# Fadi987/PL-BERT

Measured on AMD Instinct MI355X. Metric: phoneme-tokens/sec, higher is better.
Workload: dtype bf16; 1 GPU; PL-BERT masked-phoneme training step (fwd+loss+bwd+allreduce+AdamW), ALBERT hidden 768 / 12 shared layers / FFN 2048 / 12 heads, seq_len 512, batch 32 per GPU; global_batch=32, seq_len=512, parallelism=dp1

## Files before the change

include/plbert.h:

```cpp
#ifndef PLBERT_H
#define PLBERT_H

#include <stdint.h>

#ifdef __cplusplus
extern "C" {
#endif

typedef struct PlbEngine PlbEngine;

typedef struct {
  int32_t vocab_size;
  int32_t embedding_size;
  int32_t hidden_size;
  int32_t num_attention_heads;
  int32_t intermediate_size;
  int32_t num_hidden_layers;
  int32_t max_position_embeddings;
  int32_t type_vocab_size;
  float layer_norm_eps;
  int32_t num_phonemes;
  int32_t num_tokens;
  int32_t max_batch;
  int32_t max_seq;
// ... 50 lines not shown

int plb_loss_fwd_bwd(PlbEngine* e, const int64_t* masked_ids, const int64_t* labels, const int32_t* lengths,
                     const int32_t* idx_offsets, const int32_t* idx_flat, int32_t n_masked, int32_t B, int32_t S,
                     float* loss, void* stream);

int plb_loss_fwd(PlbEngine* e, const int64_t* masked_ids, const int64_t* labels, const int64_t* token_ids,
                 const int32_t* lengths, const int32_t* idx_offsets, const int32_t* idx_flat, int32_t n_masked, int32_t B,
                 int32_t S, float* loss, float* loss_parts, void* stream);

int plb_loss_fwd_bwd_dual(PlbEngine* e, const int64_t* masked_ids, const int64_t* labels, const int64_t* token_ids,
                          const int32_t* lengths, const int32_t* idx_offsets, const int32_t* idx_flat, int32_t n_masked,
                          int32_t B, int32_t S, float* loss, float* loss_parts, void* stream);

int plb_adamw_step(PlbEngine* e, double lr, double beta1, double beta2, double eps, double weight_decay, int32_t step,
                   double grad_scale, void* stream);

int plb_set_fp8(PlbEngine* e, int32_t on, void* stream);
int plb_fp8_state(const PlbEngine* e, int32_t* enabled, int32_t* calibrated);
int plb_fp8_stats(PlbEngine* e, float clamped_calls[8], float worst_overshoot[8], void* stream);

int32_t plb_token_head_steps(const PlbEngine* e);
int plb_set_token_head_steps(PlbEngine* e, int32_t steps);

#define PLB_COMM_ID_BYTES 128
int plb_comm_unique_id(uint8_t id[PLB_COMM_ID_BYTES]);
int plb_comm_init(PlbEngine* e, const uint8_t id[PLB_COMM_ID_BYTES], int32_t rank, int32_t world);
int plb_comm_destroy(PlbEngine* e);
int plb_comm_info(const PlbEngine* e, int32_t* rank, int32_t* world, int32_t* rccl_version);
int plb_status(PlbEngine* e, int32_t* ln_exchange_timeouts);
int plb_status_ex(PlbEngine* e, int32_t* ln_exchange_timeouts, int32_t* skipped_updates);
int plb_poll_status(const PlbEngine* e, int32_t* ln_exchange_timeouts);
int plb_status_export(PlbEngine* e, float* out, void* stream);
int plb_status_import(PlbEngine* e, const float* summed, void* stream);
int plb_last_application_rows(const PlbEngine* e, int64_t* rows, int64_t* of);
typedef struct {
  const int32_t* row_start;
  int32_t rows;
  int32_t used;
} PlbPacking;
int plb_packing_plan(const int32_t* lengths, int32_t B, int32_t S, int32_t* row_start, int32_t* rows, int32_t* used);
int plb_forward_packed(PlbEngine* e, const int64_t* ids, const int32_t* lengths, int32_t B, int32_t S,
                       const PlbPacking* packing, float* hidden, float* phoneme_logits, float* token_logits, void* stream);
int plb_loss_fwd_bwd_packed(PlbEngine* e, const int64_t* masked_ids, const int64_t* labels, const int32_t* lengths,
                            const int32_t* idx_offsets, const int32_t* idx_flat, int32_t n_masked, int32_t B, int32_t S,
                            const PlbPacking* packing, float* loss, void* stream);
int plb_loss_fwd_packed(PlbEngine* e, const int64_t* masked_ids, const int64_t* labels, const int64_t* token_ids,
                        const int32_t* lengths, const int32_t* idx_offsets, const int32_t* idx_flat, int32_t n_masked,
                        int32_t B, int32_t S, const PlbPacking* packing, float* loss, float* loss_parts, void* stream);
int plb_last_call_rows(const PlbEngine* e, int64_t* rows, int64_t* of);
int plb_encode(PlbEngine* e, const int64_t* ids, const int32_t* lengths, int32_t B, int32_t S, const PlbPacking* packing,
               float* hidden, void* stream);
int plb_encode_bwd(PlbEngine* e, const int64_t* ids, const int32_t* lengths, int32_t B, int32_t S, const PlbPacking* packing,
                   const float* d_hidden, void* stream);
int plb_comm_pieces(const PlbEngine* e, int32_t* collectives, int64_t* floats);
int plb_broadcast_params(PlbEngine* e, int32_t root, void* stream);
int plb_set_grad_overlap(PlbEngine* e, int32_t overlap);
int plb_allreduce_grads(PlbEngine* e, void* stream);

int plb_apply_mask(const int64_t* ids, const int32_t* sample_off, const int32_t* word_off, const int32_t* word_begin,
                   const int32_t* word_len, const int8_t* action, const int64_t* repl, const int64_t* word_token,
                   int64_t sep_token, const int32_t* crop_start, int32_t B, int32_t S, int32_t mask_id, int64_t* labels,
                   int64_t* masked, int64_t* tokens, int32_t* lengths_out, int32_t* idx_offsets, int32_t* idx_flat,
                   int32_t* scratch, void* stream);

int plb_mask_batch(const int64_t* labels, const int32_t* lengths, int32_t B, int32_t S, uint64_t seed, uint32_t step,
                   float word_pred_prob, float phoneme_mask_prob, float replace_prob, int32_t mask_id, int32_t sep_id,
                   int64_t* masked, int32_t* idx_offsets, int32_t* idx_flat, int32_t* scratch, void* stream);

void plb_profile_enable(int on);
int plb_profile_num_classes(void);
const char* plb_profile_class_name(int cls);
int plb_profile_read(double* ms, int64_t* launches, double* flops, double* bytes);

void plb_debug_skip_piece(int index);
void plb_debug_ln_fault(int mode, int launches);
int plb_debug_hb_audit(PlbEngine* e, int32_t on, int32_t break_wait);
int plb_debug_hb_report(const PlbEngine* e, int64_t* checks, int32_t* violations, char* first, int32_t first_bytes);
int plb_comm_trace(PlbEngine* e, int32_t on);
int plb_comm_trace_read(PlbEngine* e, int32_t max_pieces, int32_t* n, int64_t* begin, int64_t* end, float* released_ms,
                        float* done_ms, float* tail_ms);
void plb_set_gemm_nt_tile(int tile);
void plb_set_gemm_nt_prefetch(int on);
void plb_set_attn_bwd_fused(int on);
void plb_set_prune_last(int on);

#ifdef __cplusplus
}
#endif
#endif
```

plbert_amd/_lib.py:

```python
from __future__ import annotations

import ctypes as C
import os

import torch

HERE = os.path.dirname(os.path.abspath(__file__))
LIB_PATH = os.environ.get("PLBERT_HIP_LIB") or os.path.join(HERE, "libplbert_hip.so")

PLB_PARAM_NAMES = [
    "encoder.embeddings.word_embeddings.weight",
    "encoder.embeddings.position_embeddings.weight",
    "encoder.embeddings.token_type_embeddings.weight",
    "encoder.embeddings.LayerNorm.weight",
    "encoder.embeddings.LayerNorm.bias",
    "encoder.encoder.embedding_hidden_mapping_in.weight",
    "encoder.encoder.embedding_hidden_mapping_in.bias",
    "encoder.encoder.albert_layer_groups.0.albert_layers.0.full_layer_layer_norm.weight",
    "encoder.encoder.albert_layer_groups.0.albert_layers.0.full_layer_layer_norm.bias",
    "encoder.encoder.albert_layer_groups.0.albert_layers.0.attention.query.weight",
    "encoder.encoder.albert_layer_groups.0.albert_layers.0.attention.key.weight",
    "encoder.encoder.albert_layer_groups.0.albert_layers.0.attention.value.weight",
    "encoder.encoder.albert_layer_groups.0.albert_layers.0.attention.query.bias",
    "encoder.encoder.albert_layer_groups.0.albert_layers.0.attention.key.bias",
    "encoder.encoder.albert_layer_groups.0.albert_layers.0.attention.value.bias",
    "encoder.encoder.albert_layer_groups.0.albert_layers.0.attention.dense.weight",
    "encoder.encoder.albert_layer_groups.0.albert_layers.0.attention.dense.bias",
    "encoder.encoder.albert_layer_groups.0.albert_layers.0.attention.LayerNorm.weight",
    "encoder.encoder.albert_layer_groups.0.albert_layers.0.attention.LayerNorm.bias",
    "encoder.encoder.albert_layer_groups.0.albert_layers.0.ffn.weight",
    "encoder.encoder.albert_layer_groups.0.albert_layers.0.ffn.bias",
    "encoder.encoder.albert_layer_groups.0.albert_layers.0.ffn_output.weight",
    "encoder.encoder.albert_layer_groups.0.albert_layers.0.ffn_output.bias",
    "phoneme_predictor.weight",
    "phoneme_predictor.bias",
    "encoder.pooler.weight",
    "encoder.pooler.bias",
    "token_predictor.weight",
    "token_predictor.bias",
]
PLB_NPARAM = len(PLB_PARAM_NAMES)

PUBLIC_SYMBOLS = [
    "plb_last_error", "plb_create", "plb_destroy", "plb_param_layout", "plb_workspace_bytes", "plb_bind",
    "plb_sync_weights", "plb_forward", "plb_pooler", "plb_loss_fwd_bwd", "plb_loss_fwd", "plb_loss_fwd_bwd_dual", "plb_adamw_step",
    "plb_set_fp8", "plb_fp8_state", "plb_fp8_stats", "plb_token_head_steps", "plb_set_token_head_steps", "plb_comm_unique_id", "plb_comm_init", "plb_comm_destroy",
    "plb_comm_info", "plb_comm_pieces", "plb_last_application_rows", "plb_last_call_rows",
    "plb_packing_plan", "plb_forward_packed", "plb_loss_fwd_bwd_packed", "plb_loss_fwd_packed", "plb_encode", "plb_encode_bwd", "plb_status", "plb_status_ex", "plb_poll_status", "plb_status_export", "plb_status_import", "plb_broadcast_params", "plb_set_grad_overlap", "plb_allreduce_grads", "plb_apply_mask",
    "plb_mask_batch", "plb_profile_enable", "plb_profile_num_classes", "plb_profile_class_name", "plb_profile_read",
    "plb_debug_skip_piece", "plb_debug_ln_fault", "plb_debug_hb_audit", "plb_debug_hb_report", "plb_comm_trace", "plb_comm_trace_read",
    "plb_set_gemm_nt_tile", "plb_set_gemm_nt_prefetch", "plb_set_attn_bwd_fused", "plb_set_prune_last",
]


class PlbConfig(C.Structure):
    _fields_ = [
        ("vocab_size", C.c_int32), ("embedding_size", C.c_int32), ("hidden_size", C.c_int32),
        ("num_attention_heads", C.c_int32), ("intermediate_size", C.c_int32), ("num_hidden_layers", C.c_int32),
        ("max_position_embeddings", C.c_int32), ("type_vocab_size", C.c_int32), ("layer_norm_eps", C.c_float),
        ("num_phonemes", C.c_int32), ("num_tokens", C.c_int32), ("max_batch", C.c_int32), ("max_seq", C.c_int32),
        ("inference_only", C.c_int32),
    ]


class PlbGemmNT(C.Structure):
    _fields_ = [
        ("A", C.c_void_p), ("lda", C.c_int), ("B", C.c_void_p), ("ldb", C.c_int),
        ("M", C.c_int), ("N", C.c_int), ("K", C.c_int), ("Mstore", C.c_int),
        ("bias", C.c_void_p), ("res", C.c_void_p), ("ldr", C.c_int), ("aux", C.c_void_p), ("ldaux", C.c_int),
        ("C", C.c_void_p), ("ldc", C.c_int), ("C2", C.c_void_p), ("ldc2", C.c_int), ("Cf", C.c_void_p), ("ldcf", C.c_int),
        ("colpart", C.c_void_p),
        ("ce_cols", C.c_int), ("ce_tgt", C.c_void_p), ("ce_pmax", C.c_void_p), ("ce_psum", C.c_void_p),
        ("ce_tlogit", C.c_void_p), ("ce_lse", C.c_void_p), ("ce_w", C.c_void_p),
        ("deq_a", C.c_void_p), ("deq_b", C.c_void_p), ("C8", C.c_void_p), ("ldc8", C.c_int), ("q_scale", C.c_void_p),
        ("q_amax", C.c_void_p), ("c8_bf8", C.c_int),
        ("ln_gamma", C.c_void_p), ("ln_beta", C.c_void_p), ("ln_mean", C.c_void_p), ("ln_rstd", C.c_void_p),
        ("ln_eps", C.c_float), ("ln_xchg", C.c_void_p), ("ln_err", C.c_void_p), ("ln_fault", C.c_int),
    ]


class PlbGemmTN(C.Structure):
    _fields_ = [
        ("A", C.c_void_p), ("lda", C.c_int), ("Ncols", C.c_int), ("B", C.c_void_p), ("ldb", C.c_int),
        ("Mtot", C.c_int), ("N", C.c_int), ("K", C.c_int), ("rows_per_split", C.c_int), ("splits", C.c_int),
        ("slab", C.c_void_p), ("deq_a", C.c_void_p), ("deq_b", C.c_void_p),
    ]


class PlbAttn(C.Structure):
    _fields_ = [
        ("qkv", C.c_void_p), ("ldqkv", C.c_int), ("lengths", C.c_void_p),
        ("B", C.c_int), ("S", C.c_int), ("NH", C.c_int), ("H", C.c_int), ("scale", C.c_float),
        ("ctx", C.c_void_p), ("ldctx", C.c_int), ("lse", C.c_void_p),
        ("dctx", C.c_void_p), ("lddctx", C.c_int), ("delta", C.c_void_p), ("dqkv", C.c_void_p), ("lddqkv", C.c_int),
        ("colpart", C.c_void_p), ("colpart_accumulate", C.c_int),
        ("ctx8", C.c_void_p), ("ldctx8", C.c_int), ("ctx_scale", C.c_void_p), ("ctx_amax", C.c_void_p),
        ("dqkv8", C.c_void_p), ("lddqkv8", C.c_int), ("dqkv_scale", C.c_void_p), ("dqkv_amax", C.c_void_p),
        ("qoff", C.c_void_p), ("q", C.c_void_p), ("ldq", C.c_int), ("nq_total", C.c_int), ("dq", C.c_void_p), ("lddq", C.c_int),
        ("dq8", C.c_void_p), ("lddq8", C.c_int),
        ("row_start", C.c_void_p),
    ]


class PlbEmbed(C.Structure):
    _fields_ = [
        ("ids", C.c_void_p), ("T", C.c_int), ("S", C.c_int), ("E", C.c_int), ("V", C.c_int),
        ("word", C.c_void_p), ("pos", C.c_void_p), ("type0", C.c_void_p), ("gamma", C.c_void_p), ("beta", C.c_void_p),
        ("eps", C.c_float), ("out", C.c_void_p), ("ldo", C.c_int), ("dout", C.c_void_p), ("lddo", C.c_int),
        ("dx", C.c_void_p), ("dword", C.c_void_p), ("dpos", C.c_void_p), ("partials", C.c_void_p), ("nblocks", C.c_int),
        ("row_start", C.c_void_p), ("lengths", C.c_void_p), ("B", C.c_int),
    ]


class PlbPacking(C.Structure):
    _fields_ = [("row_start", C.c_void_p), ("rows", C.c_int32), ("used", C.c_int32)]


class PlbLayerNorm(C.Structure):
    _fields_ = [
        ("x", C.c_void_p), ("ldx", C.c_int), ("gamma", C.c_void_p), ("beta", C.c_void_p), ("eps", C.c_float),
        ("y", C.c_void_p), ("ldy", C.c_int), ("mean", C.c_void_p), ("rstd", C.c_void_p),
        ("T", C.c_int), ("H", C.c_int), ("Tzero", C.c_int),
        ("dy", C.c_void_p), ("lddy", C.c_int), ("dx", C.c_void_p), ("lddx", C.c_int),
        ("partials", C.c_void_p), ("nblocks", C.c_int), ("accumulate", C.c_int),
        ("out8", C.c_void_p), ("ld8", C.c_int), ("q_scale", C.c_void_p), ("q_amax", C.c_void_p),
    ]


_lib = None


class HipLibraryMissing(RuntimeError):
    pass

# ... 18 lines not shown
    L.plb_destroy.restype = None
    L.plb_destroy.argtypes = [vp]
    L.plb_param_layout.restype = C.c_int
    L.plb_param_layout.argtypes = [vp, i64p, i64p, i64p, i64p]
    L.plb_workspace_bytes.restype = C.c_int64
    L.plb_workspace_bytes.argtypes = [vp]
    L.plb_bind.restype = C.c_int
    L.plb_bind.argtypes = [vp, vp, vp, vp, vp, vp, C.c_int64]
    L.plb_sync_weights.restype = C.c_int
    L.plb_sync_weights.argtypes = [vp, vp]
    L.plb_forward.restype = C.c_int
    L.plb_forward.argtypes = [vp, vp, vp, i32, i32, vp, vp, vp, vp]
    L.plb_loss_fwd_bwd.restype = C.c_int
    L.plb_loss_fwd_bwd.argtypes = [vp, vp, vp, vp, vp, vp, i32, i32, i32, vp, vp]
    L.plb_loss_fwd_bwd_dual.restype = C.c_int
    L.plb_loss_fwd_bwd_dual.argtypes = [vp, vp, vp, vp, vp, vp, vp, i32, i32, i32, vp, vp, vp]
    L.plb_pooler.restype = C.c_int
    L.plb_pooler.argtypes = [vp, vp, i32, i32, vp, vp]
    L.plb_loss_fwd.restype = C.c_int
    L.plb_loss_fwd.argtypes = [vp, vp, vp, vp, vp, vp, vp, i32, i32, i32, vp, vp, vp]
    L.plb_set_fp8.restype = C.c_int
    L.plb_set_fp8.argtypes = [vp, i32, vp]
    L.plb_fp8_state.restype = C.c_int
    L.plb_fp8_state.argtypes = [vp, C.POINTER(i32), C.POINTER(i32)]
    L.plb_token_head_steps.restype = i32
    L.plb_token_head_steps.argtypes = [vp]
    L.plb_set_token_head_steps.restype = C.c_int
    L.plb_set_token_head_steps.argtypes = [vp, i32]
    L.plb_comm_unique_id.restype = C.c_int
    L.plb_comm_unique_id.argtypes = [vp]
    L.plb_comm_init.restype = C.c_int
    L.plb_comm_init.argtypes = [vp, vp, i32, i32]
    L.plb_comm_destroy.restype = C.c_int
    L.plb_comm_destroy.argtypes = [vp]
    L.plb_comm_info.restype = C.c_int
    L.plb_comm_info.argtypes = [vp, C.POINTER(i32), C.POINTER(i32), C.POINTER(i32)]
    L.plb_status.restype = C.c_int
    L.plb_status.argtypes = [vp, C.POINTER(i32)]
    L.plb_status_ex.restype = C.c_int
    L.plb_status_ex.argtypes = [vp, C.POINTER(i32), C.POINTER(i32)]
    L.plb_poll_status.restype = C.c_int
    L.plb_poll_status.argtypes = [vp, C.POINTER(i32)]
    L.plb_fp8_stats.restype = C.c_int
    L.plb_fp8_stats.argtypes = [vp, C.POINTER(f32), C.POINTER(f32), vp]
    L.plb_last_application_rows.restype = C.c_int
    L.plb_last_application_rows.argtypes = [vp, i64p, i64p]
    if hasattr(L, "plb_packing_plan"):
        pk = C.POINTER(PlbPacking)
        L.plb_last_call_rows.restype = C.c_int
        L.plb_last_call_rows.argtypes = [vp, i64p, i64p]
        L.plb_packing_plan.restype = C.c_int
        L.plb_packing_plan.argtypes = [vp, i32, i32, vp, C.POINTER(i32), C.POINTER(i32)]
        L.plb_forward_packed.restype = C.c_int
        L.plb_forward_packed.argtypes = [vp, vp, vp, i32, i32, pk, vp, vp, vp, vp]
        L.plb_loss_fwd_bwd_packed.restype = C.c_int
        L.plb_loss_fwd_bwd_packed.argtypes = [vp, vp, vp, vp, vp, vp, i32, i32, i32, pk, vp, vp]
        L.plb_loss_fwd_packed.restype = C.c_int
        L.plb_loss_fwd_packed.argtypes = [vp, vp, vp, vp, vp, vp, vp, i32, i32, i32, pk, vp, vp, vp]
        L.plb_launch_ce_prepare_packed.restype = C.c_int
        L.plb_launch_ce_prepare_packed.argtypes = [vp, vp, vp, C.c_int, C.c_int, vp, vp, vp, vp, vp]
        L.plb_launch_unpack_rows.restype = C.c_int
        L.plb_launch_unpack_rows.argtypes = [vp, C.c_int, C.c_int, vp, vp, C.c_int, C.c_int, C.c_int, vp, vp]
    if hasattr(L, "plb_encode"):
        L.plb_encode.restype = C.c_int
        L.plb_encode.argtypes = [vp, vp, vp, i32, i32, C.POINTER(PlbPacking), vp, vp]
        L.plb_encode_bwd.restype = C.c_int
        L.plb_encode_bwd.argtypes = [vp, vp, vp, i32, i32, C.POINTER(PlbPacking), vp, vp]
        L.plb_launch_seed_dy.restype = C.c_int
        L.plb_launch_seed_dy.argtypes = [vp, vp, vp, C.c_int, C.c_int, C.c_int, C.c_int, vp, vp]
    L.plb_status_export.restype = C.c_int
    L.plb_status_export.argtypes = [vp, vp, vp]
    L.plb_status_import.restype = C.c_int
    L.plb_status_import.argtypes = [vp, vp, vp]
    L.plb_debug_hb_audit.restype = C.c_int
    L.plb_debug_hb_audit.argtypes = [vp, i32, i32]
    L.plb_debug_hb_report.restype = C.c_int
    L.plb_debug_hb_report.argtypes = [vp, i64p, C.POINTER(i32), C.c_char_p, i32]
    L.plb_comm_trace.restype = C.c_int
    L.plb_comm_trace.argtypes = [vp, i32]
    L.plb_comm_trace_read.restype = C.c_int
    L.plb_comm_trace_read.argtypes = [vp, i32, C.POINTER(i32), i64p, i64p, C.POINTER(f32), C.POINTER(f32), C.POINTER(f32)]
    L.plb_debug_ln_fault.restype = None
    L.plb_debug_ln_fault.argtypes = [C.c_int, C.c_int]
    L.plb_debug_skip_piece.restype = None
    L.plb_debug_skip_piece.argtypes = [C.c_int]
    L.plb_comm_pieces.restype = C.c_int
    L.plb_comm_pieces.argtypes = [vp, C.POINTER(i32), C.POINTER(C.c_int64)]
    L.plb_broadcast_params.restype = C.c_int
    L.plb_broadcast_params.argtypes = [vp, i32, vp]
    L.plb_set_grad_overlap.restype = C.c_int
    L.plb_set_grad_overlap.argtypes = [vp, i32]
    L.plb_allreduce_grads.restype = C.c_int
    L.plb_allreduce_grads.argtypes = [vp, vp]
    L.plb_apply_mask.restype = C.c_int
    L.plb_apply_mask.argtypes = [vp, vp, vp, vp, vp, vp, vp, vp, C.c_int64, vp, i32, i32, i32, vp, vp, vp, vp, vp, vp, vp, vp]
    L.plb_adamw_step.restype = C.c_int
    L.plb_adamw_step.argtypes = [vp, f64, f64, f64, f64, f64, i32, f64, vp]
    L.plb_mask_batch.restype = C.c_int
    L.plb_mask_batch.argtypes = [vp, vp, i32, i32, C.c_uint64, C.c_uint32, f32, f32, f32, i32, i32, vp, vp, vp, vp, vp]
    L.plb_profile_enable.restype = None
    L.plb_profile_enable.argtypes = [C.c_int]
    L.plb_profile_num_classes.restype = C.c_int
    L.plb_profile_num_classes.argtypes = []
    L.plb_profile_class_name.restype = C.c_char_p
    L.plb_profile_class_name.argtypes = [C.c_int]
    L.plb_profile_read.restype = C.c_int
    L.plb_profile_read.argtypes = [C.POINTER(C.c_double), i64p, C.POINTER(C.c_double), C.POINTER(C.c_double)]
    L.plb_launch_gemm_nt.restype = C.c_int
    L.plb_launch_gemm_nt.argtypes = [C.POINTER(PlbGemmNT), C.c_int, C.c_int, vp]
    L.plb_set_gemm_nt_tile.restype = None
    L.plb_set_gemm_nt_tile.argtypes = [C.c_int]
    L.plb_set_gemm_nt_prefetch.restype = None
    L.plb_set_gemm_nt_prefetch.argtypes = [C.c_int]
    L.plb_launch_gemm_nt_fp8.restype = C.c_int
    L.plb_launch_gemm_nt_fp8.argtypes = [C.POINTER(PlbGemmNT), C.c_int, C.c_int, vp]
    L.plb_launch_gemm_nt_fp8_ln.restype = C.c_int
    L.plb_launch_gemm_nt_fp8_ln.argtypes = [C.POINTER(PlbGemmNT), C.c_int, C.c_int, vp]
    L.plb_launch_gemm_nt_fp8_gelud.restype = C.c_int
    L.plb_launch_gemm_nt_fp8_gelud.argtypes = [C.POINTER(PlbGemmNT), C.c_int, C.c_int, vp]
    L.plb_launch_gemm_tn.restype = C.c_int
    L.plb_launch_gemm_tn.argtypes = [C.POINTER(PlbGemmTN), vp]
    L.plb_launch_gemm_tn_big.restype = C.c_int
    L.plb_launch_gemm_tn_big.argtypes = [C.POINTER(PlbGemmTN), vp]
    L.plb_launch_gemm_tn_fp8.restype = C.c_int
    L.plb_launch_gemm_tn_fp8.argtypes = [C.POINTER(PlbGemmTN), vp]
    L.plb_launch_reduce_slabs.restype = C.c_int
    L.plb_launch_reduce_slabs.argtypes = [vp, C.c_int, C.c_size_t, vp, C.c_int, vp]
    L.plb_launch_attn_fwd.restype = C.c_int
    L.plb_launch_attn_fwd.argtypes = [C.POINTER(PlbAttn), vp]
    L.plb_launch_gemm_nt_ln.restype = C.c_int
    L.plb_launch_gemm_nt_ln.argtypes = [C.POINTER(PlbGemmNT), C.c_int, vp]
    L.plb_launch_gemm_nt_gelud.restype = C.c_int
    L.plb_launch_gemm_nt_gelud.argtypes = [C.POINTER(PlbGemmNT), C.c_int, vp]
    L.plb_launch_attn_bwd.restype = C.c_int
    L.plb_launch_attn_bwd.argtypes = [C.POINTER(PlbAttn), vp]
    L.plb_launch_attn_bwd_fused.restype = C.c_int
    L.plb_launch_attn_bwd_fused.argtypes = [C.POINTER(PlbAttn), vp]
    L.plb_set_prune_last.restype = None
    L.plb_set_prune_last.argtypes = [C.c_int]
    L.plb_set_attn_bwd_fused.restype = None
    L.plb_set_attn_bwd_fused.argtypes = [C.c_int]
    L.plb_launch_ln_fwd.restype = C.c_int
    L.plb_launch_ln_fwd.argtypes = [C.POINTER(PlbLayerNorm), vp]
    L.plb_launch_ln_bwd.restype = C.c_int
    L.plb_launch_ln_bwd.argtypes = [C.POINTER(PlbLayerNorm), vp]
    L.plb_launch_embed_scatter.restype = C.c_int
    L.plb_launch_embed_scatter.argtypes = [C.POINTER(PlbEmbed), C.c_int, vp]
    L.plb_launch_ce_prepare.restype = C.c_int
    L.plb_launch_ce_prepare.argtypes = [vp, vp, vp, C.c_int, C.c_int, vp, vp, vp, vp]
    L.plb_launch_colsum.restype = C.c_int
    L.plb_launch_colsum.argtypes = [vp, C.c_int, C.c_size_t, C.c_int, C.c_int, vp, C.c_int, C.c_int, vp, C.c_int, vp]
    _lib = L
    return L


def profile_enable(on):
    lib().plb_profile_enable(int(bool(on)))


def profile_read():
    L = lib()
    n = L.plb_profile_num_classes()
    ms, fl, by = (C.c_double * n)(), (C.c_double * n)(), (C.c_double * n)()
    cnt = (C.c_int64 * n)()
    check(L.plb_profile_read(ms, cnt, fl, by), "plb_profile_read")
    return {L.plb_profile_class_name(i).decode(): dict(ms=ms[i], launches=int(cnt[i]), flops=fl[i], bytes=by[i])
# ... 8 lines not shown
```

plbert_amd/csrc/attn_bwd_fused.hip:

```cpp
#include "attn_common.h"

namespace {

constexpr int FB_KIMG = 0;
constexpr int FB_EXCH = 65536;
constexpr int FB_STG = FB_EXCH + 65536;
constexpr int FB_STAT = FB_STG + 16384;
constexpr int FB_TOTAL = FB_STAT + 512;

DEVI int kt_of(int key) { return ((key >> 1) & 1) | (((key >> 3) & 1) << 1); }
DEVI int du_f(int row) { return (((row >> 1) & 1) << 2) | ((row >> 2) & 1) | (((row >> 3) & 1) << 1); }

typedef float f32x4v __attribute__((ext_vector_type(4)));
#define MFMA16(a, b, c) __builtin_amdgcn_mfma_f32_16x16x32_bf16(a, b, c, 0, 0, 0)

DEVI bf16x8 join_tr(s16x4 a, s16x4 b) { return bf16x8{a[0], a[1], a[2], a[3], b[0], b[1], b[2], b[3]}; }
typedef __attribute__((address_space(3))) const bf16x8 lds_cbf16x8;
typedef uint32_t u32x2_t __attribute__((ext_vector_type(2)));
typedef __attribute__((address_space(3))) const f32x4 lds_cf32x4;
typedef __attribute__((address_space(3))) u32x2_t lds_u32x2;
DEVI bf16x8 lds_rd128(uint32_t a) { return *(lds_cbf16x8*)(uintptr_t)a; }
DEVI f32x4 lds_rdf4(uint32_t a) { return *(lds_cf32x4*)(uintptr_t)a; }
DEVI void lds_wr64(uint32_t a, uint32_t x, uint32_t y) { *(lds_u32x2*)(uintptr_t)a = u32x2_t{x, y}; }
DEVI bf16x8 lds_tr2(uint32_t a0, uint32_t a1) { return join_tr(lds_read_tr16_addr(a0), lds_read_tr16_addr(a1)); }
// ... 308 lines not shown
      DQ_PHASE((CUR) ^ 1);                                                                                       \
      DQ_STORE(it_ - 1);                                                                                         \
    }                                                                                                            \
    STAMP(2);                                                                                                    \
    if (it_ + 1 < NQ) F_STAT_STORE((CUR) ^ 1, it_ + 1);                                                          \
    STAMP(3);                                                                                                    \
    DMA_WAIT();                                                                                                  \
    __syncthreads();                                                                                             \
    STAMP(4);                                                                                                    \
  } while (0)
#if FUSED_DBG & 1024
  const unsigned long long tstart_ = __builtin_readcyclecounter();
  tl_ = tstart_;
#endif
  for (int i = 0; i <= NQ; i += 2) {
    F_ITER(0, i);
    if (i + 1 <= NQ) F_ITER(1, i + 1);
  }
#if FUSED_DBG & 1024
  if (lane == 0 && p.delta) {
    float* o_ = p.delta + ((size_t)blockIdx.x * 4 + wave) * 8;
    for (int k = 0; k < 6; ++k) o_[k] = (float)tk_[k] * 1e-3f;
    o_[6] = (float)(tl_ - tstart_) * 1e-3f;
  }
#endif

  LANE_ID(lane_e);
  const int tid_e = wave * 64 + lane_e;
  for (int r = NQ * 32 + (tid_e >> 3); r < S; r += 32) {
    if (B16) *(uint4*)(p.dqkv + (tok0 + r) * p.lddqkv + hd * 64 + (tid_e & 7) * 8) = make_uint4(0, 0, 0, 0);
    if (F8) *(uint2*)(p.dqkv8 + (tok0 + r) * p.lddqkv8 + hd * 64 + (tid_e & 7) * 8) = make_uint2(0, 0);
  }
  bf16_t* patch = (bf16_t*)(smem + FB_EXCH) + wave * (32 * 72);
  const bool accq = p.colpart_accumulate != 0;
#pragma unroll
  for (int kb = 0; kb < 4; ++kb) {
    const int key0 = wave * 128 + kb * 32;
    int rows_valid = S - key0; rows_valid = rows_valid > 32 ? 32 : rows_valid;
    float* cp = (p.colpart && wave < QT) ? p.colpart + ((size_t)(b * QT + wave) * 4 + kb) * (3 * H) + hd * 64 : nullptr;
    if (rows_valid > 0) {
      bf16_t* out = B16 ? p.dqkv + (tok0 + key0) * p.lddqkv + hd * 64 : nullptr;
      uint8_t* out8 = F8 ? p.dqkv8 + (tok0 + key0) * p.lddqkv8 + hd * 64 : nullptr;
      const Out8 ok8 = {out8 ? out8 + H : nullptr, p.lddqkv8, qs8, true}, ov8 = {out8 ? out8 + 2 * H : nullptr, p.lddqkv8, qs8, true};
      store_transposed<false, true>(dk[kb][0], dk[kb][1], p.scale, patch, out ? out + H : nullptr, p.lddqkv, rows_valid, lane_e,
                                    cp ? cp + H : nullptr, accq, F8 ? &ok8 : nullptr, &amax8);
      __builtin_amdgcn_wave_barrier();
      store_transposed<false, true>(dv[kb][0], dv[kb][1], 1.0f, patch, out ? out + 2 * H : nullptr, p.lddqkv, rows_valid, lane_e,
                                    cp ? cp + 2 * H : nullptr, accq, F8 ? &ov8 : nullptr, &amax8);
      __builtin_amdgcn_wave_barrier();
    } else if (cp && !accq) {
      cp[H + lane_e] = 0.f;
      cp[2 * H + lane_e] = 0.f;
    }
  }
  if (F8 && p.dqkv_amax) {
    amax8 = wave_max(amax8);
    if (lane_e == 0) atomic_max_abs(p.dqkv_amax, amax8, blockIdx.x * 4 + wave);
  }
  if (p.colpart) {
#pragma unroll
    for (int r = 0; r < 4; ++r) {
      float v = colq[r];
      v += __shfl_xor(v, 1, 64); v += __shfl_xor(v, 2, 64); v += __shfl_xor(v, 4, 64); v += __shfl_xor(v, 8, 64);
      colq[r] = v;
    }
    float* row0 = p.colpart + (size_t)(b * QT) * 4 * (3 * H) + hd * 64;
    if ((lane_e & 15) == 0) {
      float* d = row0 + 16 * wave + 4 * (lane_e >> 4);
#pragma unroll
      for (int r = 0; r < 4; ++r) d[r] = accq ? d[r] + colq[r] : colq[r];
    }
    if (!accq)
      for (int rr = 1 + wave; rr < 4 * QT; rr += 4) row0[(size_t)rr * (3 * H) + lane_e] = 0.f;
  }
}

}

extern "C" int plb_launch_attn_bwd_fused(const PlbAttn* p, hipStream_t stream) {
  if (p->H != p->NH * 64 || p->S < 1 || p->S > 512 || p->B < 1) return 1;
  if (p->row_start && !p->lengths) return 1;
  if (p->ldqkv % 8 || p->ldctx % 8 || p->lddctx % 8 || p->lddqkv % 8) return 1;
  if ((!p->dqkv && !p->dqkv8) || (p->dqkv8 && (!p->dqkv_scale || p->lddqkv8 % 8))) return 1;
  dim3 grid(p->NH * p->B), block(256);
  const double unit = (double)p->B * p->NH * (double)p->S * p->S * 64.0;
  const double io = 2.0 * p->B * p->S * (double)p->H;
  const int tok = plb_prof_begin(PLB_K_ATTN_BWD, stream, 8.0 * unit, 6.0 * io);
  if (p->dqkv && p->dqkv8) return 1;
  if (!p->dqkv8) hipLaunchKernelGGL(attn_bwd_fused_kernel<0>, grid, block, 0, stream, *p);
  else hipLaunchKernelGGL(attn_bwd_fused_kernel<1>, grid, block, 0, stream, *p);
  plb_prof_end(tok, stream);
  return hipGetLastError() == hipSuccess ? 0 : 2;
}
```

plbert_amd/csrc/engine.cpp:

```cpp
#include <stdarg.h>

#include <new>

#include "engine_internal.h"

static thread_local char g_err[512] = "";
int fail(const char* fmt, ...) {
  va_list ap;
  va_start(ap, fmt);
  vsnprintf(g_err, sizeof(g_err), fmt, ap);
  va_end(ap);
  return 1;
}
extern "C" const char* plb_last_error(void) { return g_err; }

static void layout_params(PlbEngine* e) {
  const int64_t V = e->V, E = e->E, H = e->H, I = e->I, P = e->P, NP = e->NP, NT = e->NT;
  int64_t sz[PLB_NPARAM];
  sz[PLB_WORD_EMB] = V * E; sz[PLB_POS_EMB] = P * E; sz[PLB_TYPE_EMB] = (int64_t)e->c.type_vocab_size * E;
  sz[PLB_EMB_LN_W] = E; sz[PLB_EMB_LN_B] = E;
  sz[PLB_MAP_W] = H * E; sz[PLB_MAP_B] = H;
  sz[PLB_LN2_W] = H; sz[PLB_LN2_B] = H;
  sz[PLB_Q_W] = sz[PLB_K_W] = sz[PLB_V_W] = H * H;
  sz[PLB_Q_B] = sz[PLB_K_B] = sz[PLB_V_B] = H;
// ... 23 lines not shown
    return o;
  }
};
}

extern "C" int plb_create(const PlbConfig* cfg, PlbEngine** out) {
  if (!cfg || !out) return fail("plb_create: null argument");
  const PlbConfig& c = *cfg;
  if (c.hidden_size != c.num_attention_heads * 64) return fail("plb_create: head_dim must be 64 (hidden %d, heads %d)", c.hidden_size, c.num_attention_heads);
  if (c.embedding_size % 64 || c.embedding_size > 256) return fail("plb_create: embedding_size must be a multiple of 64, <= 256");
  if (c.hidden_size % 128 || c.hidden_size > 1024) return fail("plb_create: hidden_size must be a multiple of 128, <= 1024");
  if (c.intermediate_size % 128) return fail("plb_create: intermediate_size must be a multiple of 128");
  if (c.num_phonemes < 4 || c.num_phonemes % 4 || c.num_phonemes > 256) return fail("plb_create: num_phonemes must be a multiple of 4 in [4,256]");
  if (c.num_tokens < 0 || c.num_tokens % 4) return fail("plb_create: num_tokens must be a non-negative multiple of 4");
  if (c.max_seq < 1 || c.max_seq > c.max_position_embeddings) return fail("plb_create: max_seq must be in [1, max_position_embeddings]");
  if (c.max_batch < 1 || c.num_hidden_layers < 1 || c.vocab_size < 1 || c.type_vocab_size < 1) return fail("plb_create: bad sizes");
  PlbEngine* e = new (std::nothrow) PlbEngine();
  if (!e) return fail("plb_create: out of host memory");
  e->c = c;
  e->E = c.embedding_size; e->H = c.hidden_size; e->I = c.intermediate_size; e->L = c.num_hidden_layers;
  e->NH = c.num_attention_heads; e->V = c.vocab_size; e->P = c.max_position_embeddings;
  e->NP = c.num_phonemes; e->NT = c.num_tokens;
  layout_params(e);
  const int64_t E = e->E, H = e->H, I = e->I, L = e->L;
  const int64_t T = (int64_t)c.max_batch * c.max_seq;
  const int64_t Tp = rup(T, 128);
  e->infer = c.inference_only != 0;
  const bool tr = !e->infer;
  const int64_t Ls = tr ? L : 1;
  e->Tcap = Tp;
  e->NMcap = Tp;
  e->ln_blocks = 512;
  if (const char* v = getenv("PLBERT_LN_BLOCKS")) { const int n = atoi(v); if (n >= 64 && n <= 4096) e->ln_blocks = n; }
  e->emb_blocks = 2048;
  if (const char* v = getenv("PLBERT_LN_FUSE"))
    e->ln_fuse = !strcmp(v, "off") ? 0 : !strcmp(v, "fwd") ? 1 : !strcmp(v, "bwd") ? 2 : 3;
  e->part_rows = e->ln_blocks > (int)(2 * Tp / 128) ? e->ln_blocks : (int)(2 * Tp / 128);
  if (const char* v = getenv("PLBERT_GELU_STASH")) e->gelu_dstash_on = strcmp(v, "u") != 0;
  if (const char* v = getenv("PLBERT_FP8_TN")) e->fp8_tn = strcmp(v, "0") != 0;
  if (const char* v = getenv("PLBERT_HB_AUDIT")) e->hb.on = strcmp(v, "0") != 0;
  Carve cv;
  e->o_wbf = cv.take((e->ptotal + 256 * (H > I ? H : I)) * 2);
  if (tr) {
    e->o_wqkvT = cv.take(rup(H, 128) * 3 * H * 2);
    e->o_wdT = cv.take(rup(H, 128) * H * 2);
    e->o_w1T = cv.take(rup(H, 128) * I * 2);
    e->o_w2T = cv.take(rup(I, 128) * H * 2);
    e->o_wpT = cv.take(rup(H, 128) * 256 * 2);
    e->o_winT = cv.take(rup(E, 128) * H * 2);
  }
  e->o_e = cv.take(Tp * E * 2);
  e->o_x = cv.take((tr ? L + 1 : 2) * Tp * H * 2);
  e->o_qkv = cv.take(Ls * Tp * 3 * H * 2);
  e->o_ctx = cv.take(Ls * Tp * H * 2);
  e->o_pre1 = cv.take(Ls * Tp * H * 2);
  e->o_a = cv.take(Ls * Tp * H * 2);
  e->o_u = cv.take(Ls * Tp * I * 2);
  e->o_g = cv.take(Ls * Tp * I * 2);
  e->o_pre2 = cv.take(Ls * Tp * H * 2);
  const int64_t stat = (int64_t)c.max_batch * e->NH * c.max_seq * 4;
  e->o_lse = cv.take(Ls * stat);
  e->o_mean1 = cv.take(Ls * Tp * 4); e->o_rstd1 = cv.take(Ls * Tp * 4);
  e->o_mean2 = cv.take(Ls * Tp * 4); e->o_rstd2 = cv.take(Ls * Tp * 4);
  e->lnx_bytes = (Tp / 128) * 16 * 128 * 2 * 8;
  e->o_lnx = cv.take(e->lnx_bytes);
  e->o_lnerr = cv.take(256);
  if (tr) {
    e->o_delta = cv.take(stat);
    e->o_dqkv = cv.take(L * Tp * 3 * H * 2);
    e->o_dpre1 = cv.take(L * Tp * H * 2);
    e->o_du = cv.take(L * Tp * I * 2);
    e->o_dpre2 = cv.take(L * Tp * H * 2);
    e->o_dy0 = cv.take(Tp * H * 2); e->o_dy1 = cv.take(Tp * H * 2);
    e->o_da = cv.take(Tp * H * 2); e->o_dctx = cv.take(Tp * H * 2);
    e->o_de = cv.take(Tp * E * 2);
  }
  const int64_t NM = e->NMcap;
  e->o_hm = cv.take(NM * H * 2);
  e->o_logm = cv.take(NM * 256 * 4);
  e->o_dlog = cv.take(NM * 256 * 2);
  e->o_rows = cv.take(NM * 4); e->o_tgt = cv.take(NM * 4); e->o_w = cv.take(NM * 4); e->o_lrows = cv.take(NM * 4);
  if (tr) {
    e->o_dhm = cv.take(NM * H * 2);
    int64_t slab = 0;
    {
      const int64_t Mtot = L * Tp;
      const int ntp = (int)rup(e->NT, 256);
      const int shapes[7][2] = {{(int)(3 * H), (int)H}, {(int)H, (int)H}, {(int)I, (int)H}, {(int)H, (int)I}, {(int)H, (int)E}, {e->NP, (int)H}, {ntp, (int)H}};
      for (int i = 0; i < (e->NT ? 7 : 6); ++i) {
        int rps;
        const int64_t mt = i < 4 ? Mtot : Tp;
        const int s = tn_splits(mt, shapes[i][0], shapes[i][1], &rps);
        const int64_t f = (int64_t)s * shapes[i][0] * shapes[i][1];
        if (f > slab) slab = f;
      }
    }
    e->slab_floats = slab;
    e->o_slab = cv.take(slab * 4);
    e->o_part1 = cv.take(L * e->part_rows * 3 * H * 4);
    e->o_part2 = cv.take(L * e->part_rows * 3 * H * 4);
    e->o_parte = cv.take((int64_t)e->emb_blocks * 2 * E * 4);
    e->o_dxe = cv.take(Tp * E * 4);
    e->o_ducol = cv.take(L * (2 * Tp / 128) * I * 4);
    e->qkvcol_rows = c.max_batch * ((c.max_seq + 127) / 128) * 4;
    e->o_qkvcol = cv.take((int64_t)L * e->qkvcol_rows * 3 * H * 4);
    e->o_scratch = cv.take(512 * (3 * H > I ? 3 * H : I) * 4);
    e->o_scratch2 = cv.take(512 * (3 * H > I ? 3 * H : I) * 4);
    {
      int rps;
      const int s2 = tn_splits(Tp, (int)H, (int)E, &rps);
      e->slab2_floats = (int64_t)s2 * H * E;
      e->o_slab2 = cv.take(e->slab2_floats * 4);
    }
  }
  if (e->NT) {
    const int64_t NTp = rup(e->NT, 256);
    e->NTp = (int)NTp;
    e->o_bt = cv.take(NTp * 4);
    e->o_tlrows = cv.take(Tp * 4);
    e->o_tpmax = cv.take(Tp * (NTp / 256) * 4);
    e->o_tpsum = cv.take(Tp * (NTp / 256) * 4);
    e->o_ttl = cv.take(Tp * 4); e->o_tlse = cv.take(Tp * 4); e->o_tw = cv.take(Tp * 4);
    e->o_ttgt = cv.take(Tp * 8);
    e->o_tloss = cv.take(256);
    if (tr) {
      e->o_wtT = cv.take(rup(H, 128) * NTp * 2);
      e->o_tdl = cv.take(Tp * NTp * 2);
      e->o_tscr = cv.take(32 * NTp * 4);
      e->o_tcolp = cv.take(2 * (Tp / 128) * NTp * 4);
      e->o_tgrad = cv.take(NTp * H * 4);
    }
  }
  e->o_x8 = cv.take(Ls * Tp * H); e->o_a8 = cv.take(Ls * Tp * H); e->o_g8 = cv.take(Ls * Tp * I); e->o_c8 = cv.take(Ls * Tp * H);
  e->o_wq8 = cv.take(rup(3 * H, 128) * H + 256 * H);
  e->o_wd8 = cv.take(rup(H, 128) * H + 256 * H);
  e->o_w18 = cv.take(rup(I, 128) * H + 256 * H);
  e->o_w28 = cv.take(rup(H, 128) * I + 256 * I);
  if (tr) {
    e->o_dp8 = cv.take(L * Tp * H); e->o_du8 = cv.take(L * Tp * I); e->o_dp18 = cv.take(L * Tp * H); e->o_dq8 = cv.take(L * Tp * 3 * H);
    e->o_w2T8 = cv.take(rup(I, 128) * H + 256 * H);
    e->o_w1T8 = cv.take(rup(H, 128) * I + 256 * I);
    e->o_wqT8 = cv.take(rup(H, 128) * 3 * H + 256 * 3 * H);
    e->o_wdT8 = cv.take(rup(H, 128) * H + 256 * H);
  }
  e->f8n = 8 * (int)L + 8;
  e->o_f8amax = cv.take((int64_t)e->f8n * 64 * 16 * 4); e->o_f8scale = cv.take(e->f8n * 4); e->o_f8deq = cv.take(e->f8n * 4);
  e->o_f8stats = cv.take(8 * 8 * 4);
  e->ws_bytes = cv.off;
  *out = e;
  return 0;
}

extern "C" void plb_destroy(PlbEngine* e) {
  if (!e) return;
  (void)plb_comm_destroy(e);
  if (e->ev_fork) (void)hipEventDestroy(e->ev_fork);
  if (e->ev_join) (void)hipEventDestroy(e->ev_join);
  if (e->side) (void)hipStreamDestroy(e->side);
  if (e->host_err) (void)hipHostFree(e->host_err);
  for (auto& t : e->trace) { (void)hipEventDestroy(t.released); (void)hipEventDestroy(t.done); }
  for (auto ev : e->trace_pool) (void)hipEventDestroy(ev);
  for (auto ev : {e->tr_call0, e->tr_tail0, e->tr_tail1}) if (ev) (void)hipEventDestroy(ev);
  delete e;
}

extern "C" int plb_param_layout(const PlbEngine* e, int64_t* offsets, int64_t* sizes, int64_t* total, int64_t* trainable) {
  if (!e) return fail("plb_param_layout: null engine");
  for (int i = 0; i < PLB_NPARAM; ++i) {
    if (offsets) offsets[i] = e->poff[i];
    if (sizes) sizes[i] = e->psize[i];
  }
  if (total) *total = e->ptotal;
  if (trainable) *trainable = e->ptrain;
  return 0;
}

extern "C" int64_t plb_workspace_bytes(const PlbEngine* e) { return e ? e->ws_bytes : -1; }

extern "C" int plb_bind(PlbEngine* e, float* params, float* grads, float* exp_avg, float* exp_avg_sq, void* workspace,
                        int64_t workspace_bytes) {
  if (!e || !params || !workspace) return fail("plb_bind: null argument");
  if (workspace_bytes < e->ws_bytes) return fail("plb_bind: workspace too small (%lld < %lld)", (long long)workspace_bytes, (long long)e->ws_bytes);
  if (((uintptr_t)params | (uintptr_t)grads | (uintptr_t)exp_avg | (uintptr_t)exp_avg_sq) & 15) return fail("plb_bind: buffers must be 16-byte aligned");
  if ((uintptr_t)workspace & 255) return fail("plb_bind: workspace must be 256-byte aligned");
  e->params = params; e->grads = grads; e->m = exp_avg; e->v = exp_avg_sq;
  e->ws = (char*)workspace;
  if (!e->host_err) {
    void* h = nullptr;
    if (hipHostMalloc(&h, 64, hipHostMallocMapped) == hipSuccess && h) {
      void* d = nullptr;
      if (hipHostGetDevicePointer(&d, h, 0) == hipSuccess && d) {
        e->host_err = (unsigned int*)h;
        e->host_err_dev = (unsigned int*)d;
        *e->host_err = 0;
      } else {
        (void)hipHostFree(h);
      }
    }
    if (!e->host_err) return fail("plb_bind: cannot allocate the pinned status word");
  }
  if (!e->side && grads && !getenv("PLBERT_NO_SIDE_STREAM")) {
    if (hipStreamCreateWithFlags(&e->side, hipStreamNonBlocking) != hipSuccess) e->side = nullptr;
    if (e->side && (hipEventCreateWithFlags(&e->ev_fork, kStreamOrderEvent) != hipSuccess ||
                    hipEventCreateWithFlags(&e->ev_join, kStreamOrderEvent) != hipSuccess)) {
      (void)hipStreamDestroy(e->side);
      e->side = nullptr;
    }
  }
  return 0;
}

static int sync_transposes(PlbEngine* e, hipStream_t s, bool exact_fp8 = true) {
  const int H = e->H, I = e->I, E = e->E;

  if (e->NT) {
    if (!e->tok_pad_zeroed) HIPTRY(hipMemsetAsync(e->at<float>(e->o_bt), 0, (size_t)e->NTp * 4, s));
    HIPTRY(hipMemcpyAsync(e->at<float>(e->o_bt), e->par(PLB_TOK_B), (size_t)e->NT * 4, hipMemcpyDeviceToDevice, s));
  }
  if (e->infer) {
    e->tok_pad_zeroed = true;
    if (e->fp8_on) return fp8_quantize_weights(e, s, exact_fp8 || e->fp8_wstale);
    return 0;
  }
  const float* tsrc[8] = {e->par(PLB_Q_W), e->par(PLB_DENSE_W), e->par(PLB_FFN_W), e->par(PLB_FFNO_W), e->par(PLB_HEAD_W),
                          e->par(PLB_MAP_W)};
  bf16_t* tdst[8] = {e->at<bf16_t>(e->o_wqkvT), e->at<bf16_t>(e->o_wdT), e->at<bf16_t>(e->o_w1T), e->at<bf16_t>(e->o_w2T),
                     e->at<bf16_t>(e->o_wpT), e->at<bf16_t>(e->o_winT)};
  int tR[8] = {3 * H, H, I, H, e->NP, H}, tC[8] = {H, H, H, I, H, E}, tld[8] = {3 * H, H, I, H, 256, H};
  int nt = 6;
  if (e->NT) {
    if (!e->tok_pad_zeroed) HIPTRY(hipMemsetAsync(e->at<bf16_t>(e->o_wtT), 0, (size_t)rup(H, 128) * e->NTp * 2, s));
    tsrc[nt] = e->par(PLB_TOK_W); tdst[nt] = e->at<bf16_t>(e->o_wtT); tR[nt] = e->NT; tC[nt] = H; tld[nt] = e->NTp;
    ++nt;
  }
  TRY(plb_launch_transpose_cast_multi(nt, tsrc, tR, tC, tdst, tld, s));
  e->tok_pad_zeroed = true;
  if (e->fp8_on) return fp8_quantize_weights(e, s, exact_fp8 || e->fp8_wstale);
  return 0;
}

extern "C" int plb_sync_weights(PlbEngine* e, void* stream) {
  if (!e || !e->ws) return fail("plb_sync_weights: engine not bound");
  drop_stash(e, "plb_sync_weights refreshed the compute copies since");
  hipStream_t s = (hipStream_t)stream;
  TRY(plb_launch_cast_bf16(e->params, e->at<bf16_t>(e->o_wbf), (size_t)e->ptotal, s));
  return sync_transposes(e, s);
}

extern "C" int plb_pooler(PlbEngine* e, const float* hidden, int32_t B, int32_t S, float* pooled, void* stream) {
  if (!e || !e->ws) return fail("plb_pooler: engine not bound");
  if (!hidden || !pooled || B < 1 || S < 1) return fail("plb_pooler: bad argument");
  TRY(plb_launch_pooler(hidden, B, S, e->H, e->par(PLB_POOL_W), e->par(PLB_POOL_B), pooled, (hipStream_t)stream));
  return 0;
}

#ifndef PLB_PACK_GRAN_MAX
#define PLB_PACK_GRAN_MAX 1024
#endif
extern "C" int plb_packing_plan(const int32_t* lengths, int32_t B, int32_t S, int32_t* row_start, int32_t* rows,
                                int32_t* used) {
// ... 112 lines not shown
```

plbert_amd/csrc/engine_calls.cpp:

```cpp
#include "engine_internal.h"

void drop_stash(PlbEngine* e, const char* by) {
  if (e && e->stash_live) { e->stash_live = false; e->stash_dead_by = by; }
}

static int check_shape(const PlbEngine* e, int B, int S, const char* who) {
  if (!e || !e->ws) return fail("%s: engine not bound", who);
  if (B < 1 || S < 1 || B > e->c.max_batch || S > e->c.max_seq || (int64_t)B * S > (int64_t)e->c.max_batch * e->c.max_seq)
    return fail("%s: batch %d x seq %d exceeds the engine capacity %d x %d", who, B, S, e->c.max_batch, e->c.max_seq);
  return 0;
}

static Rows padded_rows(int B, int S) { return Rows{nullptr, B * S, rup(B * S, 128)}; }
static int pick_rows(PlbEngine* e, const PlbPacking* pk, const int32_t* lengths, bool dual, int B, int S, const char* who,
                     Rows* out) {
  *out = padded_rows(B, S);
  e->last_exec_rows[0] = e->last_exec_rows[1] = (int64_t)B * S;
  if (!pk || !pk->row_start) return 0;
  if (pk->rows < 128 || pk->rows % 128 || pk->used < 1 || pk->used > pk->rows)
    return fail("%s: packing plan of %d rows (%d used) is not one plb_packing_plan made", who, pk->rows, pk->used);
  if (pk->rows > out->Tp) return fail("%s: packing plan of %d rows exceeds the call's %lld", who, pk->rows, (long long)out->Tp);
  if (!lengths || dual || e->fp8_on || pk->rows == out->Tp) return 0;
  if (pk->used % 128) return fail("%s: packing plan with %d used rows: slots are multiples of 128", who, pk->used);
  *out = Rows{pk->row_start, pk->used, pk->rows};
// ... 225 lines not shown
  } else {
    HB_R(s2, st.du, Mtot_c * I * 2, "dU of every application");
    TRY(plb_launch_colsum(st.du, 1, (size_t)Mtot_c, I, I, e->grd(PLB_FFN_B), I, 0, scratch2, 64, s2));
  }
  const size_t prow = (size_t)L * e->part_rows_used;
  HB_R(s2, st.part1, (int64_t)L * e->part_rows * 3 * H * 4, "LayerNorm-1 backward partial rows");
  HB_W(s2, e->grd(PLB_DENSE_B), 3 * H * 4, "dense.bias + LayerNorm-1 affine gradients");
  TRY(plb_launch_colsum(st.part1, 0, prow, 3 * H, 3 * H, e->grd(PLB_LN1_W), 2 * H, 0, scratch2, 64, s2));
  TRY(plb_launch_copy_cols(scratch2, 64, 3 * H, 2 * H, H, e->grd(PLB_DENSE_B), s2));
  HB_R(s2, st.part2, (int64_t)L * e->part_rows * 3 * H * 4, "LayerNorm-2 backward partial rows");
  HB_W(s2, e->grd(PLB_LN2_W), 2 * H * 4, "LayerNorm-2 affine gradients"); HB_W(s2, e->grd(PLB_FFNO_B), H * 4, "ffn_output.bias gradient");
  TRY(plb_launch_colsum(st.part2, 0, prow, 3 * H, 3 * H, e->grd(PLB_LN2_W), 2 * H, 0, scratch2, 64, s2));
  TRY(plb_launch_copy_cols(scratch2, 64, 3 * H, 2 * H, H, e->grd(PLB_FFNO_B), s2));
  if (s2 != s) HIPTRY(ev_record(e, e->ev_join, s2));
  const bool ov = overlapping(e);
  const bool t8 = e->tn8_call;
  float* const slab = e->at<float>(e->o_slab);
  HB_W(s, slab, e->slab_floats * 4, "weight-gradient slab"); HB_W(s, e->grd(PLB_Q_W), 3 * H * H * 4, "Q/K/V weight gradients");
  if (t8 ? weight_grad8(e, st.dq8, st.x8, Mtot, 3 * H, H, F8_DQ, F8_X, e->grd(PLB_Q_W), s)
         : weight_grad(e, st.dqkv, 3 * H, 3 * H, st.x, H, Mtot, 3 * H, H, e->grd(PLB_Q_W), s)) return 1;
  if (ov && reduce_pieces(e, kPieceQkvW, kPieceFfnW, s)) return 1;
  HB_W(s, slab, e->slab_floats * 4, "weight-gradient slab"); HB_W(s, e->grd(PLB_FFN_W), (int64_t)I * H * 4, "ffn.weight gradient");
  if (t8 ? weight_grad8(e, st.du8, st.a8, Mtot_c, I, H, F8_DU, F8_A, e->grd(PLB_FFN_W), s)
         : weight_grad(e, st.du, I, I, st.a, H, Mtot_c, I, H, e->grd(PLB_FFN_W), s)) return 1;
  if (ov && reduce_pieces(e, kPieceFfnW, kPieceSmall, s)) return 1;
  if (ov) {
    if (reduce_pieces(e, kPieceSmall, kPieceFfnoW, s2)) return 1;
  }
  HB_W(s, slab, e->slab_floats * 4, "weight-gradient slab"); HB_W(s, e->grd(PLB_FFNO_W), (int64_t)I * H * 4, "ffn_output.weight gradient");
  if (t8 ? weight_grad8(e, st.dp8, st.g8, Mtot_c, H, I, F8_DP, F8_G, e->grd(PLB_FFNO_W), s)
         : weight_grad(e, st.dpre2, H, H, st.g, I, Mtot_c, H, I, e->grd(PLB_FFNO_W), s)) return 1;
  if (ov && reduce_pieces(e, kPieceFfnoW, kPieceDenseW, s)) return 1;
  HB_W(s, slab, e->slab_floats * 4, "weight-gradient slab"); HB_W(s, e->grd(PLB_DENSE_W), (int64_t)H * H * 4, "dense.weight gradient");
  if (t8 ? weight_grad8(e, st.dp18, st.c8, Mtot_c, H, H, F8_DP1, F8_C, e->grd(PLB_DENSE_W), s)
         : weight_grad(e, st.dpre1, H, H, st.ctx, H, Mtot_c, H, H, e->grd(PLB_DENSE_W), s)) return 1;
  if (ov && reduce_pieces(e, kPieceDenseW, kNPieces, s)) return 1;
  return 0;
}

static int backward_tail(PlbEngine* e, const int64_t* masked_ids, const int32_t* lengths, bf16_t* dy, int B, int S,
                         const Rows& rw, int du_rows, hipStream_t s) {
  hipStream_t s2 = s;
  float* scratch2 = e->at<float>(e->o_scratch);
  HB_W(s, e->ws, e->ws_bytes, "layer loop (whole workspace)");
  if (e->trace_on) (void)hipEventRecord(e->tr_tail0, s);
  if (e->side) {
    s2 = e->side;
    scratch2 = e->at<float>(e->o_scratch2);
    HIPTRY(ev_record(e, e->ev_fork, s));
    HIPTRY(ev_wait(e, s2, e->ev_fork));
  }
  const int rc = backward_tail_streams(e, masked_ids, lengths, dy, B, S, rw, du_rows, s, s2, scratch2);
  if (s2 != s) {
    if (rc) (void)ev_record(e, e->ev_join, s2);
    const hipError_t je = ev_wait(e, s, e->ev_join);
    if (!rc && je != hipSuccess) return fail("plb_loss_fwd_bwd: joining the side stream: %s", hipGetErrorString(je));
  }
  if (e->trace_on) { (void)hipEventRecord(e->tr_tail1, s); e->tr_tail_valid = true; }
  if (rc) return rc;
  HB_W(s, e->ws, e->ws_bytes, "after the side stream's join (whole workspace)");
  return pieces_done(e);
}

static int loss_impl(PlbEngine* e, bool backward, const int64_t* masked_ids, const int64_t* labels,
                     const int64_t* token_targets, const int32_t* lengths, const int32_t* idx_offsets,
                     const int32_t* idx_flat, int32_t n_masked, int32_t B, int32_t S, const PlbPacking* pk, float* loss,
                     float* loss_parts, void* stream) {
  const char* who = backward ? "plb_loss_fwd_bwd" : "plb_loss_fwd";
  if (check_shape(e, B, S, who)) return 1;
  drop_stash(e, "a plb_loss_* call rewrote the workspace since");
  if (backward && e->infer) return fail("%s: inference-only engine (PlbConfig.inference_only = 1)", who);
  if (backward && !e->grads) return fail("%s: no gradient buffer bound", who);
  if (!masked_ids || !labels || !idx_offsets || !loss) return fail("%s: null argument", who);
  if (n_masked < 0 || n_masked > e->NMcap) return fail("%s: n_masked %d out of range", who, n_masked);
  if (token_targets && !e->NT) return fail("%s: the engine has no token head (num_tokens = 0)", who);
  hipStream_t s = (hipStream_t)stream;
  Rows rw;
  if (pick_rows(e, pk, lengths, token_targets != nullptr, B, S, who, &rw)) return 1;
  const int64_t Tp = rw.Tp;
  if (backward && begin_training_call(e, token_targets != nullptr, s)) return 1;
  if (n_masked == 0 && !token_targets) return zero_loss_call(e, backward, loss, s);

  const int NM = (int)rup(n_masked, 128);
  Prune pr = {e->at<int32_t>(e->o_rows), n_masked, NM};
  const bool prune = prune_enabled() && n_masked > 0 && !token_targets && e->L >= 2 && 2 * (int64_t)NM <= Tp;
  if (n_masked > 0) {
    if (rw.row_start)
      TRY(plb_launch_ce_prepare_packed(idx_offsets, idx_flat, labels, B, S, rw.row_start, e->at<int32_t>(e->o_rows),
                                       e->at<int32_t>(e->o_tgt), e->at<float>(e->o_w), s));
    else
      TRY(plb_launch_ce_prepare(idx_offsets, idx_flat, labels, B, S, e->at<int32_t>(e->o_rows), e->at<int32_t>(e->o_tgt),
                                e->at<float>(e->o_w), s));
  }
  if (backward) e->pruned_rows = prune ? NM : 0;
  e->last_app_rows[0] = prune ? NM : Tp; e->last_app_rows[1] = Tp;
  bf16_t* xL = nullptr;
  if (run_encoder(e, masked_ids, lengths, B, S, rw, backward, &xL, s, prune ? &pr : nullptr)) return 1;
  bf16_t* dy = backward ? e->at<bf16_t>(e->o_dy0) : nullptr;
  if (phoneme_head(e, backward, prune, xL, n_masked, Tp, dy, loss, s)) return 1;
  if (loss_parts) HIPTRY(hipMemcpyAsync(loss_parts, loss, sizeof(float), hipMemcpyDeviceToDevice, s));
  if (token_targets && token_head(e, backward, xL, token_targets, lengths, B, S, dy, loss, loss_parts, s)) return 1;
  if (!backward) {
    if (e->fp8_on) {
      TRY(fp8_update_scales(e, s));
      e->fp8_ready = true;
    }
    e->last_loss = loss;
    TRY(plb_launch_step_status(e->at<unsigned int>(e->o_lnerr), loss, e->host_err_dev, nullptr, s));
    return 0;
  }

  int du_rows = 0;
  if (encoder_bwd(e, prune ? &pr : nullptr, lengths, B, S, rw, &dy, &du_rows, s)) return 1;
  if (status_exchange(e, s)) return 1;
  if (backward_tail(e, masked_ids, lengths, dy, B, S, rw, du_rows, s)) return 1;
  if (e->fp8_on) {
    TRY(fp8_update_scales(e, s));
    e->fp8_ready = true;
    e->fp8_bwd_ready = true;
  }
  return status_finish(e, loss, s);
}

extern "C" int plb_loss_fwd_bwd(PlbEngine* e, const int64_t* masked_ids, const int64_t* labels, const int32_t* lengths,
                                const int32_t* idx_offsets, const int32_t* idx_flat, int32_t n_masked, int32_t B,
                                int32_t S, float* loss, void* stream) {
  return loss_impl(e, true, masked_ids, labels, nullptr, lengths, idx_offsets, idx_flat, n_masked, B, S, nullptr, loss, nullptr,
                   stream);
}
extern "C" int plb_loss_fwd_bwd_packed(PlbEngine* e, const int64_t* masked_ids, const int64_t* labels, const int32_t* lengths,
                                       const int32_t* idx_offsets, const int32_t* idx_flat, int32_t n_masked, int32_t B,
                                       int32_t S, const PlbPacking* packing, float* loss, void* stream) {
  return loss_impl(e, true, masked_ids, labels, nullptr, lengths, idx_offsets, idx_flat, n_masked, B, S, packing, loss, nullptr,
                   stream);
}

extern "C" int plb_loss_fwd_bwd_dual(PlbEngine* e, const int64_t* masked_ids, const int64_t* labels,
                                     const int64_t* token_ids, const int32_t* lengths, const int32_t* idx_offsets,
                                     const int32_t* idx_flat, int32_t n_masked, int32_t B, int32_t S, float* loss,
                                     float* loss_parts, void* stream) {
  if (!token_ids) return fail("plb_loss_fwd_bwd_dual: token_ids is null");
  return loss_impl(e, true, masked_ids, labels, token_ids, lengths, idx_offsets, idx_flat, n_masked, B, S, nullptr, loss,
                   loss_parts, stream);
}

extern "C" int plb_loss_fwd(PlbEngine* e, const int64_t* masked_ids, const int64_t* labels, const int64_t* token_ids,
                            const int32_t* lengths, const int32_t* idx_offsets, const int32_t* idx_flat, int32_t n_masked,
                            int32_t B, int32_t S, float* loss, float* loss_parts, void* stream) {
  return loss_impl(e, false, masked_ids, labels, token_ids, lengths, idx_offsets, idx_flat, n_masked, B, S, nullptr, loss,
                   loss_parts, stream);
}
extern "C" int plb_loss_fwd_packed(PlbEngine* e, const int64_t* masked_ids, const int64_t* labels, const int64_t* token_ids,
                                   const int32_t* lengths, const int32_t* idx_offsets, const int32_t* idx_flat,
                                   int32_t n_masked, int32_t B, int32_t S, const PlbPacking* packing, float* loss,
                                   float* loss_parts, void* stream) {
  return loss_impl(e, false, masked_ids, labels, token_ids, lengths, idx_offsets, idx_flat, n_masked, B, S, packing, loss,
                   loss_parts, stream);
}

extern "C" int plb_encode(PlbEngine* e, const int64_t* ids, const int32_t* lengths, int32_t B, int32_t S,
                          const PlbPacking* pk, float* hidden, void* stream) {
  if (check_shape(e, B, S, "plb_encode")) return 1;
  if (e->infer) return fail("plb_encode: inference-only engine (PlbConfig.inference_only = 1): a differentiable forward keeps every application's activations");
  if (!e->grads) return fail("plb_encode: no gradient buffer bound");
  if (e->fp8_on) return fail("plb_encode: fp8 mode is on (the gradient sites' delayed scales belong to the pre-training loss); call plb_set_fp8(e, 0, stream) first");
  if (!ids || !hidden) return fail("plb_encode: %s is null", !ids ? "ids" : "hidden");
  hipStream_t s = (hipStream_t)stream;
  Rows rw;
  if (pick_rows(e, pk, lengths, false, B, S, "plb_encode", &rw)) return 1;
  drop_stash(e, "a plb_encode call that failed rewrote the workspace since");
  HB_W(s, e->ws, e->ws_bytes, "plb_encode (whole workspace)");
  e->last_app_rows[0] = e->last_app_rows[1] = rw.Tp;
  bf16_t* x = nullptr;
  if (run_encoder(e, ids, lengths, B, S, rw, true, &x, s)) return 1;
  if (lengths) TRY(plb_launch_unpack_rows(x, 1, e->H, rw.row_start, lengths, B, S, e->H, hidden, s));
// ... 47 lines not shown
```

plbert_amd/csrc/engine_internal.h:

```cpp
#pragma once
#include <hip/hip_runtime.h>
#include <stdint.h>
#include <stdio.h>
#include <stdlib.h>
#include <string.h>

#include <array>
#include <map>
#include <string>
#include <vector>

#include "../../include/plbert.h"
#include "plbert_kernels.h"

#pragma GCC visibility push(hidden)

int fail(const char* fmt, ...);

static const unsigned kStreamOrderEvent = hipEventDisableTiming | hipEventReleaseToDevice;

inline int64_t rup(int64_t x, int64_t m) { return (x + m - 1) / m * m; }

#define TRY(x)                                                                    \
  do {                                                                            \
    int rc_ = (x);                                                                \
    if (rc_) return fail("%s failed (rc %d) at %s:%d", #x, rc_, __FILE__, __LINE__); \
  } while (0)
#define HIPTRY(x)                                                                                   \
  do {                                                                                              \
    hipError_t e_ = (x);                                                                            \
    if (e_ != hipSuccess) return fail("%s: %s at %s:%d", #x, hipGetErrorString(e_), __FILE__, __LINE__); \
  } while (0)
#define HB_R(stream, ptr, bytes, what) do { if (e->hb.on) e->hb.access(hb_idx(e, stream), (ptr), (size_t)(bytes), false, what); } while (0)
#define HB_W(stream, ptr, bytes, what) do { if (e->hb.on) e->hb.access(hb_idx(e, stream), (ptr), (size_t)(bytes), true, what); } while (0)

typedef void* RcclComm;

struct HbAudit {
  enum { MAIN = 0, SIDE = 1, COMM = 2, NS = 3 };
  typedef std::array<uint64_t, NS> VC;
  struct Acc { const char* what; uintptr_t a, b; int st; uint64_t tick; bool wr; };
  bool on = false;
  int break_wait = -1;
  int waits = 0;
  VC vc[NS] = {{0, 0, 0}, {0, 0, 0}, {0, 0, 0}};
  std::map<hipEvent_t, VC> ev;
  std::vector<Acc> log;
  int64_t checks = 0;
  int violations = 0;
  std::string first;
  static const char* name(int st) { return st == MAIN ? "main" : st == SIDE ? "side" : "comm"; }
  void record(hipEvent_t e, int st) { vc[st][st] += 1; ev[e] = vc[st]; }
  void wait(int st, hipEvent_t e);
  void access(int st, const void* p, size_t bytes, bool wr, const char* what);
  void new_call() { log.clear(); waits = 0; }
};

struct PlbEngine {
  PlbConfig c;
  int64_t poff[PLB_NPARAM], psize[PLB_NPARAM], ptotal, ptrain;
  int E, H, I, L, NH, V, P, NP, NT;
  int64_t Tcap;
  int64_t NMcap;
  int NTp = 0;
  bool infer = false;
  int qkvcol_rows = 0;
  int64_t slab2_floats;
  int64_t slab_floats;
  int64_t ws_bytes;
  int ln_blocks, emb_blocks;
  int part_rows = 0;
  int ln_fuse = 3;
  int64_t lnx_bytes = 0;
  bool gelu_dstash_on = true;
  bool fp8_tn = true;
  int f8n = 0;
  int64_t o_wbf, o_wqkvT, o_wdT, o_w1T, o_w2T, o_wpT, o_winT;
  int64_t o_e, o_x, o_qkv, o_ctx, o_pre1, o_a, o_u, o_g, o_pre2;
  int64_t o_lse, o_delta, o_mean1, o_rstd1, o_mean2, o_rstd2;
  int64_t o_dqkv, o_dpre1, o_du, o_dpre2;
  int64_t o_dy0, o_dy1, o_da, o_dctx, o_de;
  int64_t o_hm, o_logm, o_dlog, o_dhm, o_rows, o_tgt, o_w, o_lrows;
  int64_t o_slab, o_part1, o_part2, o_parte, o_scratch, o_dxe, o_ducol, o_slab2, o_scratch2, o_qkvcol = 0;
  int64_t o_lnx = 0, o_lnerr = 0;
  int64_t o_bt = 0, o_wtT = 0, o_tdl = 0, o_tlrows = 0, o_tscr = 0, o_tgrad = 0, o_tloss = 0;
  int64_t o_tpmax = 0, o_tpsum = 0, o_ttl = 0, o_tlse = 0, o_tw = 0, o_ttgt = 0, o_tcolp = 0;
  int64_t o_x8 = 0, o_a8 = 0, o_g8 = 0, o_c8 = 0, o_dp8 = 0, o_du8 = 0, o_dp18 = 0, o_dq8 = 0;
  int64_t o_wq8 = 0, o_wd8 = 0, o_w18 = 0, o_w28 = 0, o_w2T8 = 0, o_w1T8 = 0, o_wqT8 = 0, o_wdT8 = 0;
  int64_t o_f8amax = 0, o_f8scale = 0, o_f8deq = 0, o_f8stats = 0;
  bool fp8_on = false, fp8_ready = false, fp8_bwd_ready = false, fp8_wstale = true;
  bool u_is_derivative = false;
  bool tn8_call = false;
  int part_rows_used = 0;
  int pruned_rows = 0;
  int64_t last_app_rows[2] = {0, 0};
  int64_t last_exec_rows[2] = {0, 0};
  bool tok_grads_live = false;
  bool head_grads_live = true;
  bool tok_pad_zeroed = false;
  int tok_steps = 0;
  bool stash_live = false;
  const char* stash_dead_by = "no plb_encode has run on this engine";
  int stash_B = 0, stash_S = 0;
  int64_t stash_rows = 0, stash_used = 0;
  const int32_t* stash_row_start = nullptr;
  RcclComm comm = nullptr;
  int comm_rank = 0, comm_world = 1;
  hipStream_t comm_stream = nullptr;
  hipEvent_t ev_piece = nullptr, ev_comm_done = nullptr;
  bool overlap = true;
  bool comm_pending = false;
  bool grads_reduced = false;
  int64_t piece_floats = 0;
  int32_t piece_count = 0;
  hipEvent_t ev_status = nullptr;
  bool status_pending = false;
  int32_t status_collectives = 0;
  float* last_loss = nullptr;
  HbAudit hb;
  struct PieceTrace { int64_t a, b; hipEvent_t released, done; };
  bool trace_on = false;
  std::vector<PieceTrace> trace;
  std::vector<hipEvent_t> trace_pool;
  hipEvent_t tr_call0 = nullptr, tr_tail0 = nullptr, tr_tail1 = nullptr;
  bool tr_tail_valid = false;
  hipStream_t side = nullptr;
  hipEvent_t ev_fork = nullptr, ev_join = nullptr;
  unsigned int* host_err = nullptr;
  unsigned int* host_err_dev = nullptr;
  float *params = nullptr, *grads = nullptr, *m = nullptr, *v = nullptr;
  char* ws = nullptr;

  template <typename T>
  T* at(int64_t off) const { return reinterpret_cast<T*>(ws + off); }
  bf16_t* wbf(int which) const { return at<bf16_t>(o_wbf) + poff[which]; }
  float* par(int which) const { return params + poff[which]; }
  float* grd(int which) const { return grads + poff[which]; }
};

enum { F8_X = 0, F8_A, F8_G, F8_C, F8_DP, F8_DU, F8_DP1, F8_DQ, F8_NSITE };
enum { F8_AMAX_WORDS = 64 * 16 };
enum { F8W_QKV = 0, F8W_D, F8W_1, F8W_2, F8W_2T, F8W_1T, F8W_QKVT, F8W_DT, F8W_N };

struct Rows {
  const int32_t* row_start;
  int T; int64_t Tp;
};

struct F8Site {
  float* scale = nullptr;
  float* amax = nullptr;
  float* deq = nullptr;
  F8Site() = default;
  F8Site(const PlbEngine* e, int kind, int l);
};
struct F8Weight {
  const uint8_t* img;
  const float* deq;
  F8Weight(const PlbEngine* e, int w);
};

struct F8Op { const uint8_t* A8; const uint8_t* B8; const float* deq_a; const float* deq_b; int a_bf8; };

struct Slots {
  bf16_t *x, *y;
  bf16_t *qkv, *ctx, *pre1, *a, *u, *g, *pre2;
  float *mean1, *rstd1, *mean2, *rstd2, *lse;
  uint8_t *x8, *x8n, *c8, *a8, *g8;
  bf16_t *dqkv, *dpre1, *du, *dpre2;
  uint8_t *dp8, *du8, *dp18, *dq8;
  float *part1, *part2, *qkvcol, *ducol;
};

struct LnSlot { const float* gamma; const float* beta; const bf16_t* pre; float* mean; float* rstd; float* partials; };

struct Prune { const int32_t* rows; int n; int Mc; };

struct Bwd {
  const int32_t* lengths;
  const int32_t* row_start;
  int B, S, T;
  int64_t Tp;
  bool f8, calib;
  bool fuse_b;
  int prows;
  int du_rows;
  hipStream_t s;
};

enum { kPieceHead = 0, kPieceQkvW, kPieceFfnW, kPieceSmall, kPieceFfnoW = kPieceSmall + 5, kPieceDenseW, kNPieces };

int hb_idx(const PlbEngine* e, hipStream_t s);
hipError_t ev_record(PlbEngine* e, hipEvent_t ev, hipStream_t s);
hipError_t ev_wait(PlbEngine* e, hipStream_t s, hipEvent_t ev);
int reduce_piece(PlbEngine* e, int64_t a, int64_t b, hipStream_t after);
bool overlapping(const PlbEngine* e);
int pieces_done(PlbEngine* e);
int64_t piece_begin(const PlbEngine* e, int i);
int64_t piece_end(const PlbEngine* e, int i);
int reduce_pieces(PlbEngine* e, int from, int to, hipStream_t after);
int status_exchange(PlbEngine* e, hipStream_t s);
int status_finish(PlbEngine* e, float* loss, hipStream_t s);
int f8_site(const PlbEngine* e, int site, int l);
float* f8_deq(const PlbEngine* e, int i);
int fp8_quantize_weights(PlbEngine* e, hipStream_t s, bool exact = true);
int fp8_update_scales(PlbEngine* e, hipStream_t s);
bool f8_call(const PlbEngine* e, int64_t Tp, bool train);
bool tn8_ok(const PlbEngine* e, int64_t Mtot);
PlbGemmNT nt_desc(const bf16_t* A, const bf16_t* B, int64_t M, int N, int K);
int qkvcol_rows(int B, int S);
Slots slots(const PlbEngine* e, int64_t Tp, int B, int S, int l, bool stash, int prows = 0, int du_rows = 0);
bool prune_enabled();
int run_encoder(PlbEngine* e, const int64_t* ids, const int32_t* lengths, int B, int S, const Rows& rw, bool stash,
                bf16_t** xout, hipStream_t s, const Prune* pr = nullptr);
int tn_splits(int64_t Mtot, int N, int K, int* rows_per_split);
int weight_grad(PlbEngine* e, const bf16_t* A, int lda, int Ncols, const bf16_t* Bm, int ldb, int64_t Mtot, int N,
                int K, float* out, hipStream_t s, bool side_slab = false);
int weight_grad8(PlbEngine* e, const uint8_t* A8, const uint8_t* B8, int64_t Mtot, int N, int K, int site_a, int site_b,
                 float* out, hipStream_t s);
int encoder_bwd(PlbEngine* e, const Prune* pr, const int32_t* lengths, int B, int S, const Rows& rw, bf16_t** dy,
                int* du_rows, hipStream_t s);
void drop_stash(PlbEngine* e, const char* by);

#pragma GCC visibility pop
```

plbert_amd/csrc/engine_layers.cpp:

```cpp
#include "engine_internal.h"

static bool tn_big(int64_t Mtot, int Ncols, int K) { return Ncols % 256 == 0 && K % 256 == 0 && Mtot >= 8192; }
static bool tn_fill_chip() {
  static const bool v = [] { const char* e = getenv("PLBERT_TN_SPLITS"); return !(e && !strcmp(e, "xcd")); }();
  return v;
}
static int tn_cus() {
  static const int v = [] {
    const char* e = getenv("PLBERT_TN_CUS");
    const int n = e ? atoi(e) : 256;
    return (n >= 64 && n <= 256) ? n : 256;
  }();
  return v;
}
int tn_splits(int64_t Mtot, int N, int K, int* rows_per_split) {
  const bool big = tn_big(Mtot, N, K);
  const int tiles = big ? (N / 256) * (K / 256) : ((N + 127) / 128) * ((K + 127) / 128);
  int splits = 768 / tiles;
  if (big) {
    int s = 32 / tiles;
    if (s < 1) s = 1;
    splits = tiles >= 256 ? 1 : (tn_fill_chip() ? (tn_cus() / tiles > 0 ? tn_cus() / tiles : 1) : 8 * s);
  }
  const int64_t maxs = Mtot / 64;
// ... 58 lines not shown
    v.dqkv = bf(e->o_dqkv, 3 * H); v.dpre1 = bf(e->o_dpre1, H); v.du = bf(e->o_du, I); v.dpre2 = bf(e->o_dpre2, H);
    v.dp8 = u8(e->o_dp8, H); v.du8 = u8(e->o_du8, I); v.dp18 = u8(e->o_dp18, H); v.dq8 = u8(e->o_dq8, 3 * H);
    v.part1 = f32(e->o_part1, (int64_t)prows * 3 * H); v.part2 = f32(e->o_part2, (int64_t)prows * 3 * H);
    v.qkvcol = f32(e->o_qkvcol, (int64_t)qkvcol_rows(B, S) * 3 * H); v.ducol = f32(e->o_ducol, (int64_t)du_rows * I);
  }
  return v;
}

static bool ln_fusable(const PlbEngine* e, int64_t Tp, int bit) {
  const int H = e->H;
  return (e->ln_fuse & bit) && Tp % 1024 == 0 && (H % 384 == 0 ? H / 384 : H % 256 == 0 ? H / 256 : 99) <= 4;
}
static bool gelu_dstash(PlbEngine* e, int64_t Tp, bool f8_call) {
  e->u_is_derivative = e->gelu_dstash_on && (f8_call ? Tp % 128 == 0 : Tp % 256 == 0) && e->I % 256 == 0;
  return e->u_is_derivative;
}
static void ln_fields(const PlbEngine* e, PlbGemmNT* g, const float* gamma, const float* beta, float* mean, float* rstd) {
  g->ln_gamma = gamma; g->ln_beta = beta; g->ln_mean = mean; g->ln_rstd = rstd; g->ln_eps = e->c.layer_norm_eps;
  g->ln_xchg = e->at<unsigned long long>(e->o_lnx); g->ln_err = e->at<unsigned int>(e->o_lnerr);
}
static LnSlot ln1_slot(const PlbEngine* e, const Slots& v) {
  return LnSlot{e->par(PLB_LN1_W), e->par(PLB_LN1_B), v.pre1, v.mean1, v.rstd1, v.part1};
}
static LnSlot ln2_slot(const PlbEngine* e, const Slots& v) {
  return LnSlot{e->par(PLB_LN2_W), e->par(PLB_LN2_B), v.pre2, v.mean2, v.rstd2, v.part2};
}
static int gemm_ln_fwd(PlbEngine* e, PlbGemmNT* g, const F8Op* f8, bool fused, const LnSlot& ln, bf16_t* y, int T,
                       uint8_t* y8, const F8Site& q, hipStream_t s) {
  const int H = e->H;
  if (fused) {
    g->C2 = y; g->ldc2 = H;
    ln_fields(e, g, ln.gamma, ln.beta, ln.mean, ln.rstd);
    if (y8) f8_out(g, y8, H, q, 0);
    TRY(gemm_nt_ln_any(g, 5, f8, s));
    return 0;
  }
  TRY(gemm_nt_any(g, 0, f8, s));
  PlbLayerNorm p;
  memset(&p, 0, sizeof(p));
  p.x = g->C; p.ldx = H; p.gamma = ln.gamma; p.beta = ln.beta; p.eps = e->c.layer_norm_eps;
  p.y = y; p.ldy = H; p.T = T; p.H = H; p.mean = ln.mean; p.rstd = ln.rstd;
  if (y8) { p.out8 = y8; p.ld8 = H; p.q_scale = q.scale; p.q_amax = q.amax; }
  TRY(plb_launch_ln_fwd(&p, s));
  return 0;
}
static int ln_bwd(PlbEngine* e, const LnSlot& ln, int nblocks, const bf16_t* dy, bf16_t* dx, int T, int Tzero, uint8_t* dx8,
                  const F8Site& q, hipStream_t s) {
  const int H = e->H;
  PlbLayerNorm p;
  memset(&p, 0, sizeof(p));
  p.x = ln.pre; p.ldx = H; p.gamma = ln.gamma; p.T = T; p.H = H; p.Tzero = Tzero; p.mean = ln.mean; p.rstd = ln.rstd;
  p.dy = dy; p.lddy = H; p.dx = dx; p.lddx = H; p.partials = ln.partials; p.nblocks = nblocks;
  if (dx8) { p.out8 = dx8; p.ld8 = H; p.q_scale = q.scale; p.q_amax = q.amax; }
  TRY(plb_launch_ln_bwd(&p, s));
  return 0;
}
static int gemm_ln_bwd(PlbEngine* e, PlbGemmNT* g, const F8Op* f8, bool fused, const LnSlot& ln, int nblocks, bf16_t* dx, int T,
                       int Tzero, uint8_t* dx8, const F8Site& q, hipStream_t s) {
  if (fused) {
    g->C = dx; g->aux = ln.pre; g->ldaux = e->H; g->colpart = ln.partials;
    ln_fields(e, g, ln.gamma, nullptr, ln.mean, ln.rstd);
    if (dx8) f8_out(g, dx8, e->H, q, 1);
    TRY(gemm_nt_ln_any(g, 6, f8, s));
    return 0;
  }
  TRY(gemm_nt_any(g, 0, f8, s));
  return ln_bwd(e, ln, nblocks, g->C, dx, T, Tzero, dx8, q, s);
}

static int g_prune_last = -1;
extern "C" void plb_set_prune_last(int on) { g_prune_last = on < 0 ? -1 : (on ? 1 : 0); }
bool prune_enabled() {
  static const bool v = [] { const char* e = getenv("PLBERT_PRUNE_LAST"); return !(e && !strcmp(e, "0")); }();
  return g_prune_last < 0 ? v : g_prune_last != 0;
}
static int last_application_fwd_pruned(PlbEngine* e, const Prune* pr, bool stash, bool calib, bool tn8, const Slots& sl,
                                       const bf16_t* ctx_att, hipStream_t s) {
  const int H = e->H, I = e->I, L = e->L, Mc = pr->Mc, n = pr->n;
  const F8Site sA(e, F8_A, L - 1), sG(e, F8_G, L - 1), sC(e, F8_C, L - 1);
  bf16_t* ctxc = stash ? sl.ctx : sl.pre1;
  bf16_t* xc = stash ? e->at<bf16_t>(e->o_da) : sl.a;
  bf16_t* pre1c = stash ? sl.pre1 : sl.ctx;
  bf16_t* ac = stash ? sl.a : sl.pre1;
  TRY(plb_launch_gather_rows(ctx_att, H, pr->rows, n, Mc, H, ctxc, H, s));
  TRY(plb_launch_gather_rows(sl.x, H, pr->rows, n, Mc, H, xc, H, s));
  PlbGemmNT g = nt_desc(ctxc, e->wbf(PLB_DENSE_W), Mc, H, H);
  g.bias = e->par(PLB_DENSE_B); g.res = xc; g.ldr = H; g.C = pre1c; g.ldc = H;
  const LnSlot ln1 = {e->par(PLB_LN1_W), e->par(PLB_LN1_B), pre1c, sl.mean1, sl.rstd1, nullptr};
  if (gemm_ln_fwd(e, &g, nullptr, false, ln1, ac, Mc, nullptr, F8Site(), s)) return 1;
  if (calib) TRY(plb_launch_amax(ac, 1, (size_t)n, H, H, sA.amax, s));
  g = nt_desc(ac, e->wbf(PLB_FFN_W), Mc, I, H);
  g.bias = e->par(PLB_FFN_B); g.C = sl.u; g.ldc = I; g.C2 = sl.g; g.ldc2 = I;
  TRY(plb_launch_gemm_nt(&g, 1, 0, s));
  if (calib) TRY(plb_launch_amax(sl.g, 1, (size_t)n, I, I, sG.amax, s));
  g = nt_desc(sl.g, e->wbf(PLB_FFNO_W), Mc, H, I);
  g.bias = e->par(PLB_FFNO_B); g.res = ac; g.ldr = H; g.C = sl.pre2; g.ldc = H;
  if (gemm_ln_fwd(e, &g, nullptr, false, ln2_slot(e, sl), e->at<bf16_t>(e->o_hm), Mc, nullptr, F8Site(), s)) return 1;
  if (tn8) {
    const void* src[3] = {ctxc, ac, sl.g}; const int fl[3] = {1, 1, 1};
    const size_t nel[3] = {(size_t)Mc * H, (size_t)Mc * H, (size_t)Mc * I};
    const float* sc[3] = {sC.scale, sA.scale, sG.scale};
    uint8_t* dst[3] = {sl.c8, sl.a8, sl.g8};
    float* am[3] = {sC.amax, sA.amax, sG.amax};
    TRY(plb_launch_quantize_multi(3, src, fl, nel, sc, dst, am, s));
  }
  return 0;
}

int run_encoder(PlbEngine* e, const int64_t* ids, const int32_t* lengths, int B, int S, const Rows& rw, bool stash,
                       bf16_t** xout, hipStream_t s, const Prune* pr) {
  const int E = e->E, H = e->H, I = e->I, L = e->L;
  const int T = rw.T;
  const int64_t Tp = rw.Tp;
  const bool f8 = f8_call(e, Tp, stash);
  const bool calib = e->fp8_on && !f8;
  if (e->fp8_on && e->fp8_wstale) TRY(fp8_quantize_weights(e, s));
  PlbEmbed em;
  memset(&em, 0, sizeof(em));
  em.ids = ids; em.T = T; em.S = S; em.E = E; em.V = e->V;
  em.word = e->par(PLB_WORD_EMB); em.pos = e->par(PLB_POS_EMB); em.type0 = e->par(PLB_TYPE_EMB);
  em.gamma = e->par(PLB_EMB_LN_W); em.beta = e->par(PLB_EMB_LN_B); em.eps = e->c.layer_norm_eps;
  em.out = e->at<bf16_t>(e->o_e); em.ldo = E;
  if (rw.row_start) {
    em.row_start = rw.row_start; em.lengths = lengths; em.B = B; em.T = (int)Tp;
  }
  TRY(plb_launch_embed_fwd(&em, s));

  const Slots first = slots(e, Tp, B, S, 0, stash);
  PlbGemmNT g = nt_desc(em.out, e->wbf(PLB_MAP_W), Tp, H, E);
  g.bias = e->par(PLB_MAP_B); g.C = first.x; g.ldc = H;
  TRY(plb_launch_gemm_nt(&g, 0, 0, s));
  if (f8) {
    const F8Site sX(e, F8_X, 0);
    const void* src1[1] = {first.x}; const int bf1[1] = {1}; const size_t n1[1] = {(size_t)T * H};
    const float* sc1[1] = {sX.scale}; uint8_t* dst1[1] = {first.x8}; float* am1[1] = {sX.amax};
    TRY(plb_launch_quantize_multi(1, src1, bf1, n1, sc1, dst1, am1, s));
  }
  const bool fuse_f = ln_fusable(e, Tp, 1);
  const bool dstash = gelu_dstash(e, Tp, f8);
  if (stash) e->tn8_call = f8 && e->fp8_tn && dstash && tn8_ok(e, (int64_t)L * Tp);
  const bool tn8 = stash && e->tn8_call;

  for (int l = 0; l < L; ++l) {
    const Slots sl = slots(e, Tp, B, S, l, stash);
    const F8Site sX(e, F8_X, l), sA(e, F8_A, l), sG(e, F8_G, l), sC(e, F8_C, l);
    if (calib) TRY(plb_launch_amax(sl.x, 1, (size_t)T, H, H, sX.amax, s));
    g = nt_desc(sl.x, e->wbf(PLB_Q_W), Tp, 3 * H, H);
    g.bias = e->par(PLB_Q_B); g.C = sl.qkv; g.ldc = 3 * H;
    const F8Op oq = f8_op(sl.x8, sX, F8Weight(e, F8W_QKV), 0);
    TRY(gemm_nt_any(&g, 0, f8 ? &oq : nullptr, s));
    PlbAttn at;
    memset(&at, 0, sizeof(at));
    at.qkv = sl.qkv; at.ldqkv = 3 * H; at.lengths = lengths; at.B = B; at.S = S; at.NH = e->NH; at.H = H;
    at.row_start = rw.row_start;
    const bool pruned_layer = pr != nullptr && l == L - 1;
    bf16_t* const ctx_att = (pruned_layer && stash) ? e->at<bf16_t>(e->o_dy1) : sl.ctx;
    at.scale = 0.125f; at.ctx = ctx_att; at.ldctx = H; at.lse = sl.lse;
    if (f8 && !pruned_layer) { at.ctx8 = sl.c8; at.ldctx8 = H; at.ctx_scale = sC.scale; at.ctx_amax = sC.amax; }
    TRY(plb_launch_attn_fwd(&at, s));
    if (rw.row_start && Tp > T) HIPTRY(hipMemsetAsync(ctx_att + (int64_t)T * H, 0, (size_t)(Tp - T) * H * 2, s));
    if (calib) TRY(plb_launch_amax(ctx_att, 1, (size_t)T, H, H, sC.amax, s));
    if (pruned_layer) {
      if (last_application_fwd_pruned(e, pr, stash, calib, tn8, sl, ctx_att, s)) return 1;
      *xout = e->at<bf16_t>(e->o_hm);
      break;
    }
    g = nt_desc(sl.ctx, e->wbf(PLB_DENSE_W), Tp, H, H);
    g.bias = e->par(PLB_DENSE_B); g.res = sl.x; g.ldr = H; g.C = sl.pre1; g.ldc = H;
// ... 46 lines not shown
int weight_grad8(PlbEngine* e, const uint8_t* A8, const uint8_t* B8, int64_t Mtot, int N, int K, int site_a, int site_b,
                        float* out, hipStream_t s) {
  PlbGemmTN t;
  memset(&t, 0, sizeof(t));
  t.A = reinterpret_cast<const bf16_t*>(A8); t.lda = N; t.Ncols = N; t.B = reinterpret_cast<const bf16_t*>(B8); t.ldb = K;
  t.Mtot = (int)Mtot; t.N = N; t.K = K;
  t.splits = tn_splits(Mtot, N, K, &t.rows_per_split);
  t.rows_per_split = (int)rup(t.rows_per_split, 128);
  t.splits = (int)((Mtot + t.rows_per_split - 1) / t.rows_per_split);
  if ((int64_t)t.splits * N * K > e->slab_floats) return fail("weight_grad8: slab too small");
  t.slab = e->at<float>(e->o_slab);
  t.deq_a = f8_deq(e, f8_site(e, site_a, 0)); t.deq_b = f8_deq(e, f8_site(e, site_b, 0));
  const int tok = plb_prof_begin(PLB_K_GEMM_TN_FP8, s, 2.0 * (double)Mtot * N * K, 0.0);
  TRY(plb_launch_gemm_tn_fp8(&t, s));
  plb_prof_end(tok, s);
  TRY(plb_launch_reduce_slabs(t.slab, t.splits, (size_t)N * K, out, 0, s));
  return 0;
}

static int post_attention_bwd(PlbEngine* e, const Bwd& c, int l, const Slots& sl, const bf16_t* dy) {
  const int H = e->H, I = e->I, T = c.T, Tp = (int)c.Tp;
  hipStream_t s = c.s;
  const F8Site sDP(e, F8_DP, l), sDU(e, F8_DU, l), sDP1(e, F8_DP1, l);
  if (l == e->L - 1 && ln_bwd(e, ln2_slot(e, sl), c.prows, dy, sl.dpre2, T, Tp, c.f8 ? sl.dp8 : nullptr, sDP, s)) return 1;
  if (c.calib) TRY(plb_launch_amax(sl.dpre2, 1, (size_t)T, H, H, sDP.amax, s));
  PlbGemmNT g = nt_desc(sl.dpre2, e->at<bf16_t>(e->o_w2T), Tp, I, H);
  g.aux = sl.u; g.ldaux = I; g.C = sl.du; g.ldc = I;
  if (c.du_rows > 0) g.colpart = sl.ducol;
  if (c.f8) f8_out(&g, sl.du8, I, sDU, 1);
  const F8Op ou = f8_op(sl.dp8, sDP, F8Weight(e, F8W_2T), 1);
  if (e->u_is_derivative) {
    if (e->tn8_call) g.C = nullptr;
    TRY(gemm_nt_gelud_any(&g, 1, c.f8 ? &ou : nullptr, s));
  } else {
    TRY(gemm_nt_any(&g, 2, c.f8 ? &ou : nullptr, s));
  }
  if (c.calib) TRY(plb_launch_amax(sl.du, 1, (size_t)T, I, I, sDU.amax, s));
  g = nt_desc(sl.du, e->at<bf16_t>(e->o_w1T), Tp, H, I);
  g.res = sl.dpre2; g.ldr = H; g.C = e->at<bf16_t>(e->o_da); g.ldc = H;
  const F8Op oa = f8_op(sl.du8, sDU, F8Weight(e, F8W_1T), 1);
  if (gemm_ln_bwd(e, &g, c.f8 ? &oa : nullptr, c.fuse_b, ln1_slot(e, sl), c.prows, sl.dpre1, T, Tp, c.f8 ? sl.dp18 : nullptr,
                  sDP1, s))
    return 1;
  if (c.calib) TRY(plb_launch_amax(sl.dpre1, 1, (size_t)T, H, H, sDP1.amax, s));
  g = nt_desc(sl.dpre1, e->at<bf16_t>(e->o_wdT), Tp, H, H);
  g.C = e->at<bf16_t>(e->o_dctx); g.ldc = H;
  const F8Op oc = f8_op(sl.dp18, sDP1, F8Weight(e, F8W_DT), 1);
  TRY(gemm_nt_any(&g, 0, c.f8 ? &oc : nullptr, s));
  return 0;
}

static int last_application_bwd_pruned(PlbEngine* e, const Bwd& c, const Slots& sl, const Prune* pr) {
  const int H = e->H, I = e->I, L = e->L, Mc = pr->Mc, n = pr->n;
  hipStream_t s = c.s;
  const F8Site sDP(e, F8_DP, L - 1), sDU(e, F8_DU, L - 1), sDP1(e, F8_DP1, L - 1);
  bf16_t* const dac = e->at<bf16_t>(e->o_da);
  bf16_t* const dctxc = e->at<bf16_t>(e->o_dy0);
  bf16_t* const dctx = e->at<bf16_t>(e->o_dctx);
  if (ln_bwd(e, ln2_slot(e, sl), c.prows, e->at<bf16_t>(e->o_dhm), sl.dpre2, Mc, Mc, nullptr, F8Site(), s)) return 1;
  if (c.calib) TRY(plb_launch_amax(sl.dpre2, 1, (size_t)n, H, H, sDP.amax, s));
  PlbGemmNT g = nt_desc(sl.dpre2, e->at<bf16_t>(e->o_w2T), Mc, I, H);
  g.aux = sl.u; g.ldaux = I; g.C = sl.du; g.ldc = I;
  TRY(plb_launch_gemm_nt(&g, 2, 0, s));
  if (c.calib) TRY(plb_launch_amax(sl.du, 1, (size_t)n, I, I, sDU.amax, s));
  if (c.du_rows > 0) {
    TRY(plb_launch_colsum(sl.du, 1, (size_t)Mc, I, I, sl.ducol, I, 0, e->at<float>(e->o_scratch), 16, s));
    if (c.du_rows > 1) HIPTRY(hipMemsetAsync(sl.ducol + I, 0, (size_t)(c.du_rows - 1) * I * 4, s));
  }
  g = nt_desc(sl.du, e->at<bf16_t>(e->o_w1T), Mc, H, I);
  g.res = sl.dpre2; g.ldr = H; g.C = dac; g.ldc = H;
  if (gemm_ln_bwd(e, &g, nullptr, false, ln1_slot(e, sl), c.prows, sl.dpre1, Mc, Mc, nullptr, F8Site(), s)) return 1;
  if (c.calib) TRY(plb_launch_amax(sl.dpre1, 1, (size_t)n, H, H, sDP1.amax, s));
  if (e->tn8_call) {
    const void* src[3] = {sl.dpre2, sl.du, sl.dpre1}; const int fl[3] = {3, 3, 3};
    const size_t nel[3] = {(size_t)Mc * H, (size_t)Mc * I, (size_t)Mc * H};
    const float* sc[3] = {sDP.scale, sDU.scale, sDP1.scale};
    uint8_t* dst[3] = {sl.dp8, sl.du8, sl.dp18};
    float* am[3] = {sDP.amax, sDU.amax, sDP1.amax};
    TRY(plb_launch_quantize_multi(3, src, fl, nel, sc, dst, am, s));
  }
  g = nt_desc(sl.dpre1, e->at<bf16_t>(e->o_wdT), Mc, H, H);
  g.C = dctxc; g.ldc = H;
  TRY(plb_launch_gemm_nt(&g, 0, 0, s));
  HIPTRY(hipMemsetAsync(dctx, 0, (size_t)c.Tp * H * 2, s));
  TRY(plb_launch_scatter_rows(dctxc, H, pr->rows, n, H, dctx, H, s));
  HIPTRY(hipMemsetAsync(dac, 0, (size_t)c.Tp * H * 2, s));
  TRY(plb_launch_scatter_rows(sl.dpre1, H, pr->rows, n, H, dac, H, s));
  return 0;
}

static int attention_bwd_dx(PlbEngine* e, const Bwd& c, int l, const Slots& sl, bf16_t* ctx, const bf16_t* res,
                            bf16_t* dx) {
  const int H = e->H, T = c.T;
  hipStream_t s = c.s;
  const F8Site sDQ(e, F8_DQ, l);
  PlbAttn at;
  memset(&at, 0, sizeof(at));
  at.qkv = sl.qkv; at.ldqkv = 3 * H; at.lengths = c.lengths; at.B = c.B; at.S = c.S; at.NH = e->NH; at.H = H; at.scale = 0.125f;
  at.row_start = c.row_start;
  at.ctx = ctx; at.ldctx = H; at.lse = sl.lse;
  at.dctx = e->at<bf16_t>(e->o_dctx); at.lddctx = H; at.delta = e->at<float>(e->o_delta); at.dqkv = sl.dqkv; at.lddqkv = 3 * H;
  at.colpart = sl.qkvcol; at.colpart_accumulate = 0;
  if (c.f8) {
    at.dqkv8 = sl.dq8; at.lddqkv8 = 3 * H; at.dqkv_scale = sDQ.scale; at.dqkv_amax = sDQ.amax;
    if (e->tn8_call) at.dqkv = nullptr;
  }
  if (c.row_start && c.S % 128 && at.dqkv) HIPTRY(hipMemsetAsync(sl.dqkv, 0, (size_t)T * 3 * H * 2, s));
  TRY(plb_launch_attn_bwd(&at, s));
  if (c.Tp > T) {
    if (at.dqkv) HIPTRY(hipMemsetAsync(sl.dqkv + (int64_t)T * 3 * H, 0, (size_t)(c.Tp - T) * 3 * H * 2, s));
    if (c.f8) HIPTRY(hipMemsetAsync(sl.dq8 + (int64_t)T * 3 * H, 0, (size_t)(c.Tp - T) * 3 * H, s));
  }
  if (c.calib) TRY(plb_launch_amax(sl.dqkv, 1, (size_t)T, 3 * H, 3 * H, sDQ.amax, s));
  PlbGemmNT g = nt_desc(sl.dqkv, e->at<bf16_t>(e->o_wqkvT), c.Tp, H, 3 * H);
  g.res = res; g.ldr = H; g.C = dx; g.ldc = H;
  const F8Op ox = f8_op(sl.dq8, sDQ, F8Weight(e, F8W_QKVT), 1);
  if (l == 0) {
    TRY(gemm_nt_any(&g, 0, c.f8 ? &ox : nullptr, s));
    return 0;
  }
  const Slots below = slots(e, c.Tp, c.B, c.S, l - 1, true, c.prows, c.du_rows);
  return gemm_ln_bwd(e, &g, c.f8 ? &ox : nullptr, c.fuse_b, ln2_slot(e, below), c.prows, below.dpre2, T, (int)c.Tp,
                     c.f8 ? below.dp8 : nullptr, F8Site(e, F8_DP, l - 1), s);
}

int encoder_bwd(PlbEngine* e, const Prune* pr, const int32_t* lengths, int B, int S, const Rows& rw, bf16_t** dy,
                       int* du_rows, hipStream_t s) {
  const int I = e->I, L = e->L;
  Bwd c;
  c.lengths = lengths; c.row_start = rw.row_start; c.B = B; c.S = S; c.T = rw.T; c.Tp = rw.Tp; c.s = s;
  const int Tp = (int)c.Tp;
  c.f8 = f8_call(e, Tp, true);
  c.calib = e->fp8_on && !c.f8;
  c.du_rows = e->u_is_derivative ? (c.f8 ? 2 * (Tp / plb_gemm_nt_fp8_gelud_tile_rows(Tp)) : 2 * (Tp / 256))
                                 : (c.f8 ? 2 * (Tp / 128) : plb_gemm_nt_colpart_rows(Tp, I, e->H));
  c.fuse_b = ln_fusable(e, Tp, 2);
  c.prows = c.fuse_b ? 2 * Tp / 128 : e->ln_blocks;
  e->part_rows_used = c.prows;
  bf16_t* dx = e->at<bf16_t>(e->o_dy1);
  for (int l = L - 1; l >= 0; --l) {
    const Slots sl = slots(e, c.Tp, B, S, l, true, c.prows, c.du_rows);
    if (pr && l == L - 1) {
      if (last_application_bwd_pruned(e, c, sl, pr)) return 1;
      if (attention_bwd_dx(e, c, l, sl, e->at<bf16_t>(e->o_dy1), e->at<bf16_t>(e->o_da), dx)) return 1;
    } else {
      if (post_attention_bwd(e, c, l, sl, *dy)) return 1;
      if (attention_bwd_dx(e, c, l, sl, sl.ctx, sl.dpre1, dx)) return 1;
    }
    bf16_t* tmp = *dy; *dy = dx; dx = tmp;
  }
  *du_rows = c.du_rows;
  return 0;
}
```

plbert_amd/csrc/gemm.hip:

```cpp
#include "common.h"
#include "plbert_kernels.h"
#include "gemm_epilogue.h"

namespace {

constexpr int BM = 128, BN = 128, BK = 64;

DEVI int nt_lds_off(int row, int chunk) { return row * BK + ((chunk ^ ((row >> 1) & 7)) << 3); }

template <int ACT, bool OUTF32>
__global__ __launch_bounds__(256) void gemm_nt_kernel(PlbGemmNT p) {
  __shared__ __attribute__((aligned(16))) bf16_t smem[2][2][BM * BK];
  const int tid = threadIdx.x, lane = tid & 63, wave = tid >> 6;
  const int wr = wave >> 1, wc = wave & 1;
  const int nbn = (p.N + BN - 1) / BN;
  const int nwg = gridDim.x;
  const int logical = xcd_remap(blockIdx.x, nwg);
  const int bm = logical / nbn, bn = logical % nbn;

  const int uw = __builtin_amdgcn_readfirstlane(wave);
  const int drow = lane >> 3, dch = lane & 7;
  const bf16_t* gA = p.A + (size_t)(bm * BM + uw * 32 + drow) * p.lda;
  const bf16_t* gB = p.B + (size_t)(bn * BN + uw * 32 + drow) * p.ldb;
  const size_t sa = (size_t)8 * p.lda, sb = (size_t)8 * p.ldb;
  int sch[4];
#pragma unroll
  for (int i = 0; i < 4; ++i) sch[i] = (dch ^ ((4 * i + (lane >> 4)) & 7)) * 8;
  typedef __attribute__((address_space(1))) const void* gptr_t;
  typedef __attribute__((address_space(3))) void* lptr_t;
#define NT_STAGE(st, kt)                                                                              \
  do {                                                                                                \
    _Pragma("unroll") for (int i = 0; i < 4; ++i) {                                                   \
      __builtin_amdgcn_global_load_lds((gptr_t)(gA + i * sa + (size_t)(kt) * BK + sch[i]),            \
                                       (lptr_t)&smem[st][0][(uw * 32 + i * 8) * BK], 16, 0, 0);       \
      __builtin_amdgcn_global_load_lds((gptr_t)(gB + i * sb + (size_t)(kt) * BK + sch[i]),            \
                                       (lptr_t)&smem[st][1][(uw * 32 + i * 8) * BK], 16, 0, 0);       \
    }                                                                                                 \
  } while (0)
#define NT_LANDED() asm volatile("s_waitcnt vmcnt(0)" ::: "memory")

  f32x4 acc[4][4];
#pragma unroll
  for (int i = 0; i < 4; ++i)
#pragma unroll
    for (int j = 0; j < 4; ++j) acc[i][j] = f32x4{0.f, 0.f, 0.f, 0.f};

  const int frow = lane & 15, fq = lane >> 4;
  const int fsw = (frow >> 1) & 7;
  const int offA = (wr * 64 + frow) * BK, offB = (wc * 64 + frow) * BK;
#define NT_COMPUTE(st)                                                                                   \
  do {                                                                                                   \
    const bf16_t* sA = smem[st][0];                                                                      \
    const bf16_t* sB = smem[st][1];                                                                      \
    _Pragma("unroll") for (int kk = 0; kk < 2; ++kk) {                                                   \
      const int ch = ((kk * 4 + fq) ^ fsw) << 3;                                                         \
      bf16x8 af[4], bfr[4];                                                                              \
      _Pragma("unroll") for (int i = 0; i < 4; ++i) {                                                    \
        af[i] = *(const bf16x8*)&sA[offA + i * 16 * BK + ch];                                            \
        bfr[i] = *(const bf16x8*)&sB[offB + i * 16 * BK + ch];                                           \
      }                                                                                                  \
      _Pragma("unroll") for (int mi = 0; mi < 4; ++mi)                                                   \
        _Pragma("unroll") for (int ni = 0; ni < 4; ++ni)                                                 \
          acc[mi][ni] = __builtin_amdgcn_mfma_f32_16x16x32_bf16(bfr[ni], af[mi], acc[mi][ni], 0, 0, 0);  \
    }                                                                                                    \
  } while (0)

  const int nk = p.K / BK;
  NT_STAGE(0, 0);
  NT_LANDED();
  __syncthreads();
  for (int kt = 0; kt < nk; ++kt) {
    const int cur = kt & 1;
    if (kt + 1 < nk) NT_STAGE(cur ^ 1, kt + 1);
    NT_COMPUTE(cur);
    NT_LANDED();
    __syncthreads();
  }
#undef NT_STAGE
#undef NT_LANDED
#undef NT_COMPUTE

#pragma unroll
  for (int mi = 0; mi < 4; ++mi) {
    const int m = bm * BM + wr * 64 + mi * 16 + frow;
#pragma unroll
    for (int ni = 0; ni < 4; ++ni)
      nt_epilogue<ACT, OUTF32>(p, acc[mi][ni], m, bn * BN + wc * 64 + ni * 16 + fq * 4);
  }
}

DEVI int tn_unit(int t) { return (t & 3) | (((t >> 3) & 1) << 2) | (((t >> 2) & 1) << 3) | (t & 48); }
DEVI int tn_lds_off(int t, int col) {
  int s = col >> 4;
  return s * 1024 + (((tn_unit(t) + s) & 63) << 4) + (col & 15);
}

__global__ __launch_bounds__(256) void gemm_tn_kernel(PlbGemmTN p) {
  __shared__ __attribute__((aligned(16))) bf16_t smem[2][2][64 * 128];
  const int tid = threadIdx.x, lane = tid & 63, wave = tid >> 6;
  const int wn = wave >> 1, wk = wave & 1;
  const int nbk = (p.K + 127) / 128;
  const int bn = blockIdx.x / nbk, bk = blockIdx.x % nbk;
  const int split = blockIdx.y;
  const int t_begin = split * p.rows_per_split;
  int t_end = t_begin + p.rows_per_split;
  if (t_end > p.Mtot) t_end = p.Mtot;
  const int nt = (t_end - t_begin) / 64;

  const int lc = tid & 15, lr = tid >> 4;
  const int colA = bn * 128 + lc * 8, colB = bk * 128 + lc * 8;
  const bool okA = colA < p.Ncols, okB = colB < p.K;
  uint4 ra[4], rb[4];
  auto load_tile = [&](int it) {
    const size_t t0 = (size_t)t_begin + (size_t)it * 64 + lr;
#pragma unroll
    for (int i = 0; i < 4; ++i) {
      ra[i] = okA ? *(const uint4*)(p.A + (t0 + 16 * i) * p.lda + colA) : make_uint4(0, 0, 0, 0);
      rb[i] = okB ? *(const uint4*)(p.B + (t0 + 16 * i) * p.ldb + colB) : make_uint4(0, 0, 0, 0);
    }
  };
  auto store_tile = [&](int st) {
#pragma unroll
    for (int i = 0; i < 4; ++i) {
      int off = tn_lds_off(lr + 16 * i, lc * 8);
      *(uint4*)&smem[st][0][off] = ra[i];
      *(uint4*)&smem[st][1][off] = rb[i];
    }
  };

  f32x4 acc[4][4];
#pragma unroll
  for (int i = 0; i < 4; ++i)
#pragma unroll
    for (int j = 0; j < 4; ++j) acc[i][j] = f32x4{0.f, 0.f, 0.f, 0.f};

  const int g = lane >> 4, li = lane & 15, q = li >> 2, pp = li & 3;
  if (nt > 0) {
    load_tile(0);
    store_tile(0);
  }
  __syncthreads();
  for (int it = 0; it < nt; ++it) {
    const int cur = it & 1;
    if (it + 1 < nt) load_tile(it + 1);
    const bf16_t* sA = smem[cur][0];
    const bf16_t* sB = smem[cur][1];
#pragma unroll
    for (int ks = 0; ks < 2; ++ks) {
      const int t0 = ks * 32 + 8 * g + q;
      bf16x8 af[4], bfr[4];
#pragma unroll
      for (int i = 0; i < 4; ++i) {
        const int ca = wn * 64 + i * 16 + 4 * pp, cb = wk * 64 + i * 16 + 4 * pp;
        s16x4 a0 = lds_read_tr16(&sA[tn_lds_off(t0, ca)]);
        s16x4 a1 = lds_read_tr16(&sA[tn_lds_off(t0 + 4, ca)]);
        s16x4 b0 = lds_read_tr16(&sB[tn_lds_off(t0, cb)]);
        s16x4 b1 = lds_read_tr16(&sB[tn_lds_off(t0 + 4, cb)]);
        af[i] = bf16x8{a0[0], a0[1], a0[2], a0[3], a1[0], a1[1], a1[2], a1[3]};
        bfr[i] = bf16x8{b0[0], b0[1], b0[2], b0[3], b1[0], b1[1], b1[2], b1[3]};
      }
#pragma unroll
      for (int ni = 0; ni < 4; ++ni)
#pragma unroll
        for (int ki = 0; ki < 4; ++ki)
          acc[ni][ki] = __builtin_amdgcn_mfma_f32_16x16x32_bf16(bfr[ki], af[ni], acc[ni][ki], 0, 0, 0);
    }
    if (it + 1 < nt) store_tile(cur ^ 1);
    __syncthreads();
  }

  float* out = p.slab + (size_t)split * p.N * p.K;
#pragma unroll
  for (int ni = 0; ni < 4; ++ni) {
    const int n = bn * 128 + wn * 64 + ni * 16 + li;
    if (n >= p.N) continue;
#pragma unroll
    for (int ki = 0; ki < 4; ++ki) {
      const int k0 = bk * 128 + wk * 64 + ki * 16 + 4 * g;
      if (k0 >= p.K) continue;
      f32x4 v = acc[ni][ki];
      *(float4*)(out + (size_t)n * p.K + k0) = make_float4(v[0], v[1], v[2], v[3]);
    }
  }
}

}

static int g_nt_tile = 0;
extern "C" void plb_set_gemm_nt_tile(int tile) { g_nt_tile = tile; }

static int pick_tile(const PlbGemmNT* p) {
  const bool ok256 = p->M % 256 == 0 && p->N % 256 == 0, ok384 = p->M % 128 == 0 && p->N % 384 == 0;
  const bool ok1256 = p->M % 128 == 0 && p->N % 256 == 0;
  if (g_nt_tile == 128) return 128;
  if (g_nt_tile == 256) return ok256 ? 256 : 128;
  if (g_nt_tile == 384) return ok384 ? 384 : (ok256 ? 256 : 128);
  if (g_nt_tile == 1256) return ok1256 ? 1256 : 128;
  if ((long)p->M * p->N < 256L * 256 * 64) return 128;
  double e256 = 0, e384 = 0, e1256 = 0;
  if (ok256) { const long t = (long)(p->M / 256) * (p->N / 256); e256 = (double)t / (double)(((t + 255) / 256) * 256); }
  if (ok384) { const long t = (long)(p->M / 128) * (p->N / 384); e384 = 0.95 * (double)t / (double)(((t + 255) / 256) * 256); }
  if (ok1256) { const long t = (long)(p->M / 128) * (p->N / 256); e1256 = 0.85 * (double)t / (double)(((t + 255) / 256) * 256); }
  if (e256 == 0 && e384 == 0 && e1256 == 0) return 128;
  if (e1256 > e256 && e1256 > e384) return 1256;
  return e384 > e256 ? 384 : 256;
}

extern "C" int plb_gemm_nt_colpart_rows(int M, int N, int K) {
  PlbGemmNT q;
  q.M = M; q.N = N; q.K = K;
  const int tile = pick_tile(&q);
  return tile == 256 ? 2 * (M / 256) : (tile == 384 || tile == 1256) ? 2 * (M / 128) : 0;
}

extern "C" int plb_launch_gemm_nt(const PlbGemmNT* p, int act, int out_f32, hipStream_t stream) {
  if (p->M % BM || p->K % BK || p->N % 4 || p->M <= 0 || p->N <= 0 || p->K <= 0) return 1;
  const int nbn = (p->N + BN - 1) / BN;
  dim3 grid((p->M / BM) * nbn), block(256);
  const int cls = out_f32 ? PLB_K_GEMM_NT_F32 : act == 1 ? PLB_K_GEMM_NT_GELU : act == 2 ? PLB_K_GEMM_NT_GELUBWD : PLB_K_GEMM_NT;
  const int tile = pick_tile(p);
  if (p->colpart && tile == 128) return 1;
  const double mnk = (double)p->M * p->N * p->K;
  const double algo_bytes = 2.0 * ((double)p->M * p->K + (double)p->N * p->K) +
                            (double)p->M * p->N * (out_f32 ? 4 : act == 1 ? 4 : 2) +
                            (p->res ? 2.0 * p->M * p->N : 0.0) + (act == 2 ? 2.0 * p->M * p->N : 0.0);
  if (tile != 128) {
    const int tokb = plb_prof_begin(cls, stream, 2.0 * mnk, algo_bytes);
    const int rc = plb_launch_gemm_nt_big(p, tile, act, out_f32, stream);
    plb_prof_end(tokb, stream);
    return rc;
  }
  const int tok = plb_prof_begin(out_f32 ? PLB_K_GEMM_NT_F32 : PLB_K_GEMM_NT_SMALL, stream, 2.0 * mnk, algo_bytes);
  if (out_f32) {
    if (act != 0) return 1;
    hipLaunchKernelGGL((gemm_nt_kernel<0, true>), grid, block, 0, stream, *p);
  } else if (act == 0) {
    hipLaunchKernelGGL((gemm_nt_kernel<0, false>), grid, block, 0, stream, *p);
  } else if (act == 1) {
    hipLaunchKernelGGL((gemm_nt_kernel<1, false>), grid, block, 0, stream, *p);
  } else if (act == 2) {
    hipLaunchKernelGGL((gemm_nt_kernel<2, false>), grid, block, 0, stream, *p);
  } else {
    return 1;
  }
  plb_prof_end(tok, stream);
  return hipGetLastError() == hipSuccess ? 0 : 2;
}

extern "C" int plb_launch_gemm_tn(const PlbGemmTN* p, hipStream_t stream) {
  if (p->Mtot % 64 || p->rows_per_split % 64 || p->K % 4 || p->N <= 0 || p->splits <= 0) return 1;
  if ((long)p->splits * p->rows_per_split < p->Mtot) return 1;
  dim3 grid(((p->N + 127) / 128) * ((p->K + 127) / 128), p->splits), block(256);
  const int tok = plb_prof_begin(PLB_K_GEMM_TN, stream, 2.0 * p->Mtot * (double)p->N * p->K,
                                 2.0 * p->Mtot * ((double)p->N + p->K) + 4.0 * p->splits * (double)p->N * p->K);
  hipLaunchKernelGGL(gemm_tn_kernel, grid, block, 0, stream, *p);
  plb_prof_end(tok, stream);
  return hipGetLastError() == hipSuccess ? 0 : 2;
}
```

plbert_amd/csrc/plbert_kernels.h:

```cpp
#pragma once
#include <hip/hip_runtime.h>
#include <stdint.h>

typedef uint16_t bf16_t;

extern "C" {

enum PlbKernelClass {
  PLB_K_GEMM_NT = 0, PLB_K_GEMM_NT_GELU, PLB_K_GEMM_NT_GELUBWD, PLB_K_GEMM_NT_F32, PLB_K_GEMM_TN,
  PLB_K_ATTN_FWD, PLB_K_ATTN_BWD_DQ, PLB_K_ATTN_BWD_DKV, PLB_K_LN_FWD, PLB_K_LN_BWD, PLB_K_EMBED_FWD,
  PLB_K_EMBED_BWD, PLB_K_COLSUM, PLB_K_REDUCE, PLB_K_ROWS, PLB_K_CE, PLB_K_ADAMW, PLB_K_CAST, PLB_K_TOKEN_CE, PLB_K_GEMM_NT_CE, PLB_K_GEMM_NT_SMALL, PLB_K_FP8, PLB_K_ATTN_BWD,
  PLB_K_GEMM_NT_FP8, PLB_K_GEMM_NT_GELU_FP8, PLB_K_GEMM_NT_GELUBWD_FP8,
  PLB_K_GEMM_NT_LNFWD, PLB_K_GEMM_NT_LNBWD,
  PLB_K_GEMM_NT_LNFWD_FP8, PLB_K_GEMM_NT_LNBWD_FP8, PLB_K_GEMM_TN_FP8,
  PLB_K_NCLASS
};
int plb_prof_begin(int cls, hipStream_t s, double flops, double bytes);
void plb_prof_end(int tok, hipStream_t s);

typedef struct {
  const bf16_t* A; int lda;
  const bf16_t* B; int ldb;
  int M, N, K;
  int Mstore;
// ... 45 lines not shown
} PlbGemmTN;
int plb_launch_gemm_tn(const PlbGemmTN* p, hipStream_t stream);
int plb_launch_gemm_tn_fp8(const PlbGemmTN* p, hipStream_t stream);
int plb_launch_gemm_tn_big(const PlbGemmTN* p, hipStream_t stream);

int plb_launch_reduce_slabs(const float* slab, int splits, size_t n, float* out, int accumulate, hipStream_t stream);

typedef struct {
  const int64_t* ids; int T, S, E, V;
  const float *word, *pos, *type0, *gamma, *beta;
  float eps;
  bf16_t* out; int ldo;
  const bf16_t* dout; int lddo;
  float* dx;
  float *dword, *dpos;
  float* partials;
  int nblocks;
  const int32_t* row_start; const int32_t* lengths; int B;
} PlbEmbed;
int plb_launch_embed_fwd(const PlbEmbed* p, hipStream_t stream);
int plb_launch_embed_bwd(const PlbEmbed* p, hipStream_t stream);
int plb_launch_embed_scatter(const PlbEmbed* p, int P, hipStream_t stream);

typedef struct {
  const bf16_t* x; int ldx;
  const float *gamma, *beta; float eps;
  bf16_t* y; int ldy;
  float *mean, *rstd;
  int T, H;
  int Tzero;
  const bf16_t* dy; int lddy;
  bf16_t* dx; int lddx;
  float* partials; int nblocks;
  int accumulate;
  uint8_t* out8; int ld8; const float* q_scale; float* q_amax;
} PlbLayerNorm;
int plb_launch_amax(const void* x, int is_bf16, size_t rows, int cols, int ld, float* amax, hipStream_t stream);
int plb_launch_fp8_scales(float* amax, float* scale, float* deq, int n, float fmax, int group, hipStream_t stream);
int plb_launch_fp8_scales2(float* amax, float* scale, float* deq, int n, float fmax, int group, int n2, float fmax2,
                           float* stats, int hist_from, hipStream_t stream);
int plb_launch_quantize(const void* x, int is_bf16, size_t rows, int cols, int ld, const float* scale, uint8_t* out, int ldo,
                        int bf8, hipStream_t stream);
int plb_launch_quantize_multi(int n, const void* const* src, const int* is_bf16, const size_t* elements,
                              const float* const* scale, uint8_t* const* dst, float* const* amax, hipStream_t stream);
int plb_launch_ln_fwd(const PlbLayerNorm* p, hipStream_t stream);
int plb_launch_ln_bwd(const PlbLayerNorm* p, hipStream_t stream);

int plb_launch_colsum(const void* X, int is_bf16, size_t R, int N, int ld, float* out, int Nout, int accumulate,
                      float* scratch, int nsplit, hipStream_t stream);

int plb_launch_copy_cols(const float* scratch, int nsplit, int N, int col0, int Nout, float* out, hipStream_t stream);

int plb_launch_pooler(const float* hidden, int B, int S, int H, const float* W, const float* bias, float* pooled,
                      hipStream_t stream);

typedef struct {
  const bf16_t* qkv; int ldqkv;
  const int32_t* lengths;
  int B, S, NH, H;
  float scale;
  bf16_t* ctx; int ldctx;
  float* lse;
  const bf16_t* dctx; int lddctx;
  float* delta;
  bf16_t* dqkv; int lddqkv;
  float* colpart;
  int colpart_accumulate;
  uint8_t* ctx8; int ldctx8; const float* ctx_scale; float* ctx_amax;
  uint8_t* dqkv8; int lddqkv8; const float* dqkv_scale; float* dqkv_amax;
  const int32_t* qoff; const bf16_t* q; int ldq; int nq_total; bf16_t* dq; int lddq; uint8_t* dq8; int lddq8;
  const int32_t* row_start;
} PlbAttn;
int plb_launch_attn_fwd(const PlbAttn* p, hipStream_t stream);
int plb_launch_attn_bwd(const PlbAttn* p, hipStream_t stream);
int plb_launch_attn_bwd_fused(const PlbAttn* p, hipStream_t stream);
void plb_debug_skip_piece(int index);
void plb_debug_ln_fault(int mode, int launches);
void plb_set_attn_bwd_fused(int on);

int plb_launch_gather_rows(const bf16_t* src, int lds_, const int32_t* rows, int n, int npad, int H, bf16_t* dst,
                           int ldd, hipStream_t stream);
int plb_launch_scatter_rows(const bf16_t* src, int lds_, const int32_t* rows, int n, int H, bf16_t* dst, int ldd,
                            hipStream_t stream);
int plb_launch_ce_prepare(const int32_t* offsets, const int32_t* flat, const int64_t* labels, int B, int S,
                          int32_t* rows, int32_t* tgt, float* w, hipStream_t stream);
int plb_launch_ce_prepare_packed(const int32_t* offsets, const int32_t* flat, const int64_t* labels, int B, int S,
                                 const int32_t* row_start, int32_t* rows, int32_t* tgt, float* w, hipStream_t stream);
int plb_launch_unpack_rows(const void* src, int src_is_bf16, int lds_, const int32_t* row_start, const int32_t* lengths,
                           int B, int S, int C, float* dst, hipStream_t stream);
int plb_launch_seed_dy(const float* d_hidden, const int32_t* lengths, const int32_t* row_start, int B, int S, int H, int Tp,
                       bf16_t* dy, hipStream_t stream);
int plb_launch_ce_fwd_bwd(const float* logits, int ldl, int V, const int32_t* tgt, const float* w, int n, int npad,
                          float* loss_rows, bf16_t* dlogits, int ldd, hipStream_t stream);
int plb_launch_sum_rows(const float* x, int n, float* out, hipStream_t stream);
int plb_launch_token_ce_combine(const float* pmax, const float* psum, int ntiles, const float* tlogit,
                                const int32_t* lengths, int B, int S, int rows, float* lse, float* w, float* loss_rows,
                                hipStream_t stream);
int plb_launch_add_scalar(float* out, const float* a, const float* b, hipStream_t stream);

typedef struct {
  const int64_t* labels; const int32_t* lengths;
  int B, S;
  uint64_t seed; uint32_t step;
  float word_pred_prob, mask_prob, replace_prob;
  int mask_id, sep_id;
  int64_t* masked; int32_t *counts, *idx_padded, *offsets, *flat;
} PlbMask;
int plb_launch_mask(const PlbMask* p, hipStream_t stream);

typedef struct {
  const int64_t* ids; const int32_t *sample_off, *word_off, *word_begin, *word_len; const int8_t* action;
  const int64_t* repl; const int64_t* word_token; int64_t sep_token; const int32_t* crop_start;
  int B, S, mask_id;
  int64_t *labels, *masked, *tokens; int32_t *lengths_out, *counts, *idx_padded, *offsets, *flat;
} PlbApplyMask;
int plb_launch_apply_mask(const PlbApplyMask* p, hipStream_t stream);

int plb_launch_adamw(float* p, const float* g, float* m, float* v, bf16_t* p_bf16, size_t n, double lr, double beta1,
                     double beta2, double eps, double wd, int step, double grad_scale, unsigned int* skip_if_nonzero,
                     int count_skip, hipStream_t stream);
int plb_launch_step_status(unsigned int* ln_err, float* loss, unsigned int* host_mirror, const float* summed, hipStream_t stream);
int plb_launch_status_export(const unsigned int* ln_err, float* out, hipStream_t stream);
int plb_launch_cast_bf16(const float* src, bf16_t* dst, size_t n, hipStream_t stream);
int plb_launch_transpose_cast(const float* src, int R, int C, bf16_t* dst, int ldd, hipStream_t stream);
int plb_launch_transpose_cast_multi(int n, const float* const* src, const int* R, const int* C, bf16_t* const* dst,
                                    const int* ldd, hipStream_t stream);
int plb_launch_bf16_to_f32(const bf16_t* src, int lds_, float* dst, int ldd, int R, int C, hipStream_t stream);

}
```

plbert_amd/csrc/rowops.hip:

```cpp
#include "common.h"
#include "plbert_kernels.h"

namespace {

__device__ __forceinline__ bool packed_locate(const int32_t* row_start, const int32_t* lengths, int B, int S, int r, int* b_out,
                                              int* s_out) {
  int lo = 0, hi = B;
  while (hi - lo > 1) {
    const int mid = (lo + hi) >> 1;
    if (row_start[mid] <= r) lo = mid; else hi = mid;
  }
  int len = lengths[lo];
  len = len < 1 ? 1 : (len > S ? S : len);
  *b_out = lo; *s_out = r - row_start[lo];
  return *s_out < len;
}

template <bool BWD>
__global__ __launch_bounds__(256) void embed_kernel(PlbEmbed p) {
  const int lane = threadIdx.x & 63, wave = threadIdx.x >> 6;
  const int E = p.E;
  const int c = lane * 4;
  const bool act = c < E;
  float4 g4 = make_float4(0, 0, 0, 0), b4 = g4, ty = g4;
// ... 615 lines not shown
        acc[4] += b.x; acc[5] += b.y; acc[6] += b.z; acc[7] += b.w;
      }
    }
  }
#pragma unroll
  for (int j = 0; j < 8; ++j) red[rsub][cl * 8 + j] = acc[j];
  __syncthreads();
  const int col = blockIdx.x * 256 + tid;
  if (col < N) {
    float s = 0.f;
#pragma unroll
    for (int k = 0; k < 8; ++k) s += red[k][tid];
    scratch[(size_t)blockIdx.y * N + col] = s;
  }
}

__global__ __launch_bounds__(256) void reduce_slabs_kernel(const float* slab, int splits, size_t n, float* out, int accumulate) {
  const size_t i = ((size_t)blockIdx.x * blockDim.x + threadIdx.x) * 4;
  if (i >= n) return;
  if (i + 4 <= n) {
    float4 s = accumulate ? *(const float4*)(out + i) : make_float4(0, 0, 0, 0);
    int k = 0;
    for (; k + 4 <= splits; k += 4) {
      const float4 v0 = *(const float4*)(slab + (size_t)k * n + i), v1 = *(const float4*)(slab + (size_t)(k + 1) * n + i);
      const float4 v2 = *(const float4*)(slab + (size_t)(k + 2) * n + i), v3 = *(const float4*)(slab + (size_t)(k + 3) * n + i);
      s.x = (((s.x + v0.x) + v1.x) + v2.x) + v3.x; s.y = (((s.y + v0.y) + v1.y) + v2.y) + v3.y;
      s.z = (((s.z + v0.z) + v1.z) + v2.z) + v3.z; s.w = (((s.w + v0.w) + v1.w) + v2.w) + v3.w;
    }
    for (; k < splits; ++k) {
      float4 v = *(const float4*)(slab + (size_t)k * n + i);
      s.x += v.x; s.y += v.y; s.z += v.z; s.w += v.w;
    }
    *(float4*)(out + i) = s;
  } else {
    for (size_t j = i; j < n; ++j) {
      float s = accumulate ? out[j] : 0.f;
      for (int k = 0; k < splits; ++k) s += slab[(size_t)k * n + j];
      out[j] = s;
    }
  }
}

__global__ __launch_bounds__(256) void reduce_cols_kernel(const float* scratch, int nsplit, int N, int Nout, float* out,
                                                          int accumulate, int col0) {
  __shared__ float red[8][32];
  const int c = threadIdx.x & 31, g = threadIdx.x >> 5;
  const int j = blockIdx.x * 32 + c;
  float s0 = 0.f, s1 = 0.f, s2 = 0.f, s3 = 0.f;
  if (j < Nout) {
    const float* px = scratch + col0 + j;
    int k = g;
    for (; k + 24 < nsplit; k += 32) {
      s0 += px[(size_t)k * N]; s1 += px[(size_t)(k + 8) * N]; s2 += px[(size_t)(k + 16) * N]; s3 += px[(size_t)(k + 24) * N];
    }
    for (; k < nsplit; k += 8) s0 += px[(size_t)k * N];
  }
  red[g][c] = (s0 + s1) + (s2 + s3);
  __syncthreads();
  if (g == 0 && j < Nout) {
    const float t = ((red[0][c] + red[1][c]) + (red[2][c] + red[3][c])) + ((red[4][c] + red[5][c]) + (red[6][c] + red[7][c]));
    out[j] = accumulate ? out[j] + t : t;
  }
}

__global__ void gather_rows_kernel(const bf16_t* src, int lds_, const int32_t* rows, int n, int npad, int H,
                                   bf16_t* dst, int ldd) {
  const int r = blockIdx.x;
  const int chunks = H / 8;
  const bool live = r < n;
  const size_t srow = live ? (size_t)rows[r] : 0;
  for (int c = threadIdx.x; c < chunks; c += blockDim.x) {
    uint4 v = live ? *(const uint4*)(src + srow * lds_ + c * 8) : make_uint4(0, 0, 0, 0);
    *(uint4*)(dst + (size_t)r * ldd + c * 8) = v;
  }
}
__global__ void scatter_rows_kernel(const bf16_t* src, int lds_, const int32_t* rows, int n, int H, bf16_t* dst,
                                    int ldd) {
  const int r = blockIdx.x;
  if (r >= n) return;
  const size_t drow = (size_t)rows[r];
  for (int c = threadIdx.x; c < H / 8; c += blockDim.x)
    *(uint4*)(dst + drow * ldd + c * 8) = *(const uint4*)(src + (size_t)r * lds_ + c * 8);
}
__global__ void ce_prepare_kernel(const int32_t* offsets, const int32_t* flat, const int64_t* labels, int B, int S,
                                  const int32_t* row_start, int32_t* rows, int32_t* tgt, float* w) {
  __shared__ int cnt[4];
  int c = 0;
  for (int b = threadIdx.x; b < B; b += blockDim.x) c += offsets[b + 1] > offsets[b];
  c = (int)wave_sum((float)c);
  if ((threadIdx.x & 63) == 0) cnt[threadIdx.x >> 6] = c;
  __syncthreads();
  const int count = cnt[0] + cnt[1] + cnt[2] + cnt[3];
  const int b = blockIdx.x;
  const int j0 = offsets[b], j1 = offsets[b + 1];
  const float wb = (j1 > j0) ? 1.0f / ((float)(j1 - j0) * (float)count) : 0.f;
  for (int j = j0 + threadIdx.x; j < j1; j += blockDim.x) {
    const int idx = flat[j];
    rows[j] = row_start ? row_start[b] + idx : b * S + idx;
    tgt[j] = (int32_t)labels[(size_t)b * S + idx];
    w[j] = wb;
  }
}
template <typename T>
__global__ __launch_bounds__(256) void unpack_rows_kernel(const T* src, int lds_, const int32_t* row_start, const int32_t* lengths,
                                                          int S, int C, float* dst) {
  const int b = blockIdx.x / S, s = blockIdx.x - b * S;
  int len = lengths[b];
  len = len < 1 ? 1 : (len > S ? S : len);
  float* d = dst + (size_t)blockIdx.x * C;
  if (s >= len) {
    for (int c = threadIdx.x; c < C; c += 256) d[c] = 0.f;
    return;
  }
  const T* r = src + (size_t)(row_start ? row_start[b] + s : blockIdx.x) * lds_;
  for (int c = threadIdx.x; c < C; c += 256) {
    if constexpr (sizeof(T) == 2) d[c] = bf2f(r[c]); else d[c] = r[c];
  }
}
__global__ __launch_bounds__(256) void seed_dy_kernel(const float* d_hidden, const int32_t* lengths, const int32_t* row_start, int B,
                                                      int S, int H4, unsigned int total, bf16_t* dy) {
  for (unsigned int i = blockIdx.x * 256u + threadIdx.x; i < total; i += gridDim.x * 256u) {
    const int r = (int)(i / (unsigned int)H4), c = (int)(i - (unsigned int)r * (unsigned int)H4);
    int b = 0, s = 0;
    bool live;
    if (row_start) {
      live = packed_locate(row_start, lengths, B, S, r, &b, &s);
    } else {
      b = r / S; s = r - b * S;
      live = b < B;
      if (live && lengths) { int len = lengths[b]; len = len < 1 ? 1 : (len > S ? S : len); live = s < len; }
    }
    uint2 o = make_uint2(0u, 0u);
    if (live) {
      const float4 v = *(const float4*)(d_hidden + ((size_t)b * S + s) * ((size_t)H4 * 4) + (size_t)c * 4);
      o.x = pack_bf2(v.x, v.y); o.y = pack_bf2(v.z, v.w);
    }
    *(uint2*)(dy + (size_t)i * 4) = o;
  }
}
__global__ __launch_bounds__(256) void ce_kernel(const float* logits, int ldl, int V, const int32_t* tgt, const float* w,
                                                 int n, int npad, float* loss_rows, bf16_t* dlogits, int ldd) {
  const int lane = threadIdx.x & 63, wave = threadIdx.x >> 6;
  const int r = blockIdx.x * 4 + wave;
  if (r >= npad) return;
  const int c = lane * 4;
  if (r >= n) {
    if (c < ldd) *(uint2*)(dlogits + (size_t)r * ldd + c) = make_uint2(0, 0);
    return;
  }
  float z[4];
#pragma unroll
  for (int j = 0; j < 4; ++j) z[j] = (c + j < V) ? logits[(size_t)r * ldl + c + j] : -INFINITY;
  const float mx = wave_max(fmaxf(fmaxf(z[0], z[1]), fmaxf(z[2], z[3])));
  float e[4], s = 0.f;
#pragma unroll
  for (int j = 0; j < 4; ++j) { e[j] = (c + j < V) ? __expf(z[j] - mx) : 0.f; s += e[j]; }
  s = wave_sum(s);
  const int t = tgt[r];
  const float wr = w[r];
  float zt = 0.f;
#pragma unroll
  for (int j = 0; j < 4; ++j) zt += (c + j == t) ? z[j] : 0.f;
  zt = wave_sum(zt);
  if (lane == 0) loss_rows[r] = wr * (mx + __logf(s) - zt);
  const float inv = wr / s;
  if (c < ldd) {
// ... 291 lines not shown
  if (p->H % 4 || p->H > 1024 || p->T <= 0) return 1;
  int blocks = (p->T + 4 * LN_R - 1) / (4 * LN_R); if (blocks > 4096) blocks = 4096;
  ProfScope ps(PLB_K_LN_FWD, stream, 0, (double)p->T * (4.0 * p->H + 8));
  const bool fwide_ok = (p->H == 768 || p->H == 1024) && p->ldx % 8 == 0 && p->ldy % 8 == 0;
  if (p->out8 && !fwide_ok) return 1;
  if (fwide_ok && (LN_WIDE || p->out8)) {
    const int rows_per_block = 4 * (p->H == 768 ? 2 : 1) * LNW_GROUPS;
    int wb = (p->T + rows_per_block - 1) / rows_per_block; if (wb > LNW_FWD_BLOCKS) wb = LNW_FWD_BLOCKS;
    if (p->H == 768) hipLaunchKernelGGL((ln_fwd_wide_kernel<96>), dim3(wb), dim3(256), 0, stream, *p);
    else hipLaunchKernelGGL((ln_fwd_wide_kernel<128>), dim3(wb), dim3(256), 0, stream, *p);
    return LAUNCH_OK();
  }
  const int nch = (p->H + 255) / 256;
  switch (nch) {
    case 1: hipLaunchKernelGGL((ln_fwd_kernel<1>), dim3(blocks), dim3(256), 0, stream, *p); break;
    case 2: hipLaunchKernelGGL((ln_fwd_kernel<2>), dim3(blocks), dim3(256), 0, stream, *p); break;
    case 3: hipLaunchKernelGGL((ln_fwd_kernel<3>), dim3(blocks), dim3(256), 0, stream, *p); break;
    default: hipLaunchKernelGGL((ln_fwd_kernel<4>), dim3(blocks), dim3(256), 0, stream, *p); break;
  }
  return LAUNCH_OK();
}
extern "C" int plb_launch_ln_bwd(const PlbLayerNorm* p, hipStream_t stream) {
  if (p->H % 4 || p->H > 1024 || p->T <= 0 || p->nblocks <= 0) return 1;
  ProfScope ps(PLB_K_LN_BWD, stream, 0, (double)p->T * (6.0 * p->H + 8));
  const bool wide_ok = (p->H == 768 || p->H == 1024) && p->ldx % 8 == 0 && p->lddy % 8 == 0 && p->lddx % 8 == 0;
  if (p->out8 && !wide_ok) return 1;
  if (wide_ok && (p->out8 || (LN_WIDE && p->H == 1024))) {
    if (p->H == 768) hipLaunchKernelGGL((ln_bwd_wide_kernel<96>), dim3(p->nblocks), dim3(256), 0, stream, *p);
    else hipLaunchKernelGGL((ln_bwd_wide_kernel<128>), dim3(p->nblocks), dim3(256), 0, stream, *p);
    return LAUNCH_OK();
  }
  const int nch = (p->H + 255) / 256;
  switch (nch) {
    case 1: hipLaunchKernelGGL((ln_bwd_kernel<1>), dim3(p->nblocks), dim3(256), 0, stream, *p); break;
    case 2: hipLaunchKernelGGL((ln_bwd_kernel<2>), dim3(p->nblocks), dim3(256), 0, stream, *p); break;
    case 3: hipLaunchKernelGGL((ln_bwd_kernel<3>), dim3(p->nblocks), dim3(256), 0, stream, *p); break;
    default: hipLaunchKernelGGL((ln_bwd_kernel<4>), dim3(p->nblocks), dim3(256), 0, stream, *p); break;
  }
  return LAUNCH_OK();
}
extern "C" int plb_launch_reduce_slabs(const float* slab, int splits, size_t n, float* out, int accumulate,
                                       hipStream_t stream) {
  if (!n) return 0;
  const size_t threads = (n + 3) / 4;
  ProfScope ps(PLB_K_REDUCE, stream, 0, 4.0 * (double)n * (splits + 1));
  hipLaunchKernelGGL(reduce_slabs_kernel, dim3((unsigned)((threads + 255) / 256)), dim3(256), 0, stream, slab, splits, n,
                     out, accumulate);
  return LAUNCH_OK();
}
extern "C" int plb_launch_colsum(const void* X, int is_bf16, size_t R, int N, int ld, float* out, int Nout,
                                 int accumulate, float* scratch, int nsplit, hipStream_t stream) {
  if (N % 8 || ld % 8 || nsplit <= 0 || Nout > N) return 1;
  ProfScope ps(PLB_K_COLSUM, stream, 0, (double)R * N * (is_bf16 ? 2 : 4));
  dim3 grid((N + 255) / 256, nsplit);
  if (is_bf16) hipLaunchKernelGGL((colsum_kernel<true>), grid, dim3(256), 0, stream, X, R, N, ld, scratch, nsplit);
  else hipLaunchKernelGGL((colsum_kernel<false>), grid, dim3(256), 0, stream, X, R, N, ld, scratch, nsplit);
  if (hipGetLastError() != hipSuccess) return 2;
  hipLaunchKernelGGL(reduce_cols_kernel, dim3((unsigned)((Nout + 31) / 32)), dim3(256), 0, stream, scratch, nsplit, N,
                     Nout, out, accumulate, 0);
  return LAUNCH_OK();
}
extern "C" int plb_launch_copy_cols(const float* scratch, int nsplit, int N, int col0, int Nout, float* out,
                                    hipStream_t stream) {
  if (nsplit <= 0 || col0 < 0 || col0 + Nout > N) return 1;
  hipLaunchKernelGGL(reduce_cols_kernel, dim3((unsigned)((Nout + 31) / 32)), dim3(256), 0, stream, scratch, nsplit, N,
                     Nout, out, 0, col0);
  return LAUNCH_OK();
}
extern "C" int plb_launch_gather_rows(const bf16_t* src, int lds_, const int32_t* rows, int n, int npad, int H,
                                      bf16_t* dst, int ldd, hipStream_t stream) {
  if (H % 8 || npad <= 0) return 1;
  ProfScope ps(PLB_K_ROWS, stream, 0, 4.0 * (double)npad * H);
  hipLaunchKernelGGL(gather_rows_kernel, dim3(npad), dim3(128), 0, stream, src, lds_, rows, n, npad, H, dst, ldd);
  return LAUNCH_OK();
}
extern "C" int plb_launch_scatter_rows(const bf16_t* src, int lds_, const int32_t* rows, int n, int H, bf16_t* dst,
                                       int ldd, hipStream_t stream) {
  if (H % 8) return 1;
  if (n <= 0) return 0;
  hipLaunchKernelGGL(scatter_rows_kernel
, dim3(n), dim3(128), 0, stream, src, lds_, rows, n, H, dst, ldd);
  return LAUNCH_OK();
}
extern "C" int plb_launch_ce_prepare(const int32_t* offsets, const int32_t* flat, const int64_t* labels, int B, int S,
                                     int32_t* rows, int32_t* tgt, float* w, hipStream_t stream) {
  hipLaunchKernelGGL(ce_prepare_kernel, dim3(B), dim3(256), 0, stream, offsets, flat, labels, B, S, nullptr, rows, tgt, w);
  return LAUNCH_OK();
}
extern "C" int plb_launch_ce_prepare_packed(const int32_t* offsets, const int32_t* flat, const int64_t* labels, int B, int S,
                                            const int32_t* row_start, int32_t* rows, int32_t* tgt, float* w,
                                            hipStream_t stream) {
  if (!row_start || B < 1 || S < 1) return 1;
  hipLaunchKernelGGL(ce_prepare_kernel, dim3(B), dim3(256), 0, stream, offsets, flat, labels, B, S, row_start, rows, tgt, w);
  return LAUNCH_OK();
}
extern "C" int plb_launch_unpack_rows(const void* src, int src_is_bf16, int lds_, const int32_t* row_start,
                                      const int32_t* lengths, int B, int S, int C, float* dst, hipStream_t stream) {
  if (!src || !lengths || !dst || B < 1 || S < 1 || C < 1 || lds_ < C) return 1;
  ProfScope ps(PLB_K_CAST, stream, 0, (double)B * S * C * 6.0);
  if (src_is_bf16)
    hipLaunchKernelGGL(unpack_rows_kernel<bf16_t>, dim3((unsigned)(B * S)), dim3(256), 0, stream, (const bf16_t*)src, lds_,
                       row_start, lengths, S, C, dst);
  else
    hipLaunchKernelGGL(unpack_rows_kernel<float>, dim3((unsigned)(B * S)), dim3(256), 0, stream, (const float*)src, lds_,
                       row_start, lengths, S, C, dst);
  return LAUNCH_OK();
}
extern "C" int plb_launch_seed_dy(const float* d_hidden, const int32_t* lengths, const int32_t* row_start, int B, int S, int H,
                                  int Tp, bf16_t* dy, hipStream_t stream) {
  if (!d_hidden || !dy || B < 1 || S < 1 || H < 4 || H % 4 || Tp < 1) return 1;
  if (row_start ? !lengths : (int64_t)Tp < (int64_t)B * S) return 1;
  if (((uintptr_t)d_hidden & 15) || ((uintptr_t)dy & 7)) return 1;
  const int64_t total = (int64_t)Tp * (H / 4);
  if (total >= ((int64_t)1 << 31)) return 1;
  const int64_t blocks = (total + 255) / 256;
  ProfScope ps(PLB_K_CAST, stream, 0, (double)Tp * H * 6.0);
  hipLaunchKernelGGL(seed_dy_kernel, dim3((unsigned)(blocks < 2048 ? blocks : 2048)), dim3(256), 0, stream, d_hidden, lengths,
                     row_start, B, S, H / 4, (unsigned int)total, dy);
  return LAUNCH_OK();
}
extern "C" int plb_launch_ce_fwd_bwd(const float* logits, int ldl, int V, const int32_t* tgt, const float* w, int n,
                                     int npad, float* loss_rows, bf16_t* dlogits, int ldd, hipStream_t stream) {
  if (V > 256 || ldd > 256 || ldd % 4 || npad <= 0) return 1;
  ProfScope ps(PLB_K_CE, stream, 0, (double)npad * (4.0 * V + 2.0 * ldd));
  hipLaunchKernelGGL(ce_kernel, dim3((npad + 3) / 4), dim3(256), 0, stream, logits, ldl, V, tgt, w, n, npad, loss_rows,
                     dlogits, ldd);
  return LAUNCH_OK();
}
extern "C" int plb_launch_token_ce_combine(const float* pmax, const float* psum, int ntiles, const float* tlogit,
                                           const int32_t* lengths, int B, int S, int rows, float* lse, float* w,
                                           float* loss_rows, hipStream_t stream) {
  if (ntiles < 1 || rows < B * S) return 1;
  ProfScope ps(PLB_K_TOKEN_CE, stream, 0, (double)rows * ntiles * 8.0);
  hipLaunchKernelGGL(token_ce_combine_kernel, dim3((rows + 3) / 4), dim3(256), 0, stream, pmax, psum, ntiles, tlogit, lengths,
                     B, S, rows, lse, w, loss_rows);
  return LAUNCH_OK();
}
extern "C" int plb_launch_add_scalar(float* out, const float* a, const float* b, hipStream_t stream) {
  hipLaunchKernelGGL(add_scalar_kernel, dim3(1), dim3(1), 0, stream, out, a, b);
  return LAUNCH_OK();
}
extern "C" int plb_launch_sum_rows(const float* x, int n, float* out, hipStream_t stream) {
  hipLaunchKernelGGL(sum_rows_kernel, dim3(1), dim3(256), 0, stream, x, n, out);
  return LAUNCH_OK();
}
extern "C" int plb_launch_adamw(float* p, const float* g, float* m, float* v, bf16_t* p_bf16, size_t n, double lr,
                                double beta1, double beta2, double eps, double wd, int step, double grad_scale,
                                unsigned int* skip_if_nonzero, int count_skip, hipStream_t stream) {
  if (n % 4 || step < 1) return 1;
  if (!n) return 0;
  ProfScope ps(PLB_K_ADAMW, stream, 0, (double)n * 30.0);
  const double bc1 = 1.0 - pow(beta1, step), bc2 = 1.0 - pow(beta2, step);
  hipLaunchKernelGGL(adamw_kernel, dim3((unsigned)((n / 4 + 255) / 256)), dim3(256), 0, stream, p, g, m, v, p_bf16, n,
                     (float)(1.0 - lr * wd), (float)(1.0 - beta1), (float)beta2, (float)(1.0 - beta2), (float)eps,
                     (float)(lr / bc1), (float)sqrt(bc2), (float)grad_scale, skip_if_nonzero, count_skip);
  return LAUNCH_OK();
}
extern "C" int plb_launch_step_status(unsigned int* ln_err, float* loss, unsigned int* host_mirror, const float* summed,
                                      hipStream_t stream) {
  hipLaunchKernelGGL(step_status_kernel, dim3(1), dim3(1), 0, stream, ln_err, loss, host_mirror, summed);
  return LAUNCH_OK();
}
extern "C" int plb_launch_status_export(const unsigned int* ln_err, float* out, hipStream_t stream) {
  hipLaunchKernelGGL(status_export_kernel, dim3(1), dim3(1), 0, stream, ln_err, out);
  return LAUNCH_OK();
}
// ... 84 lines not shown
```

Baseline: 1.714 million tokens/s.

## Fuse pruned-row gather/scatter passes and add 64-row GEMM tile variant

In the pruned last-layer path, the two separate row gathers become one dual-source gather launch. The two memset-plus-scatter pairs become one inverse-row-map kernel plus one fused scatter-fill kernel that writes zeros or copied rows in a single pass. This removes launches and redundant full-tensor memset writes. Separately, the small-tile NT GEMM kernel is templated on its M tile so M multiples of 64 can run with a 64-row tile, which allows padded masked-row counts and adds more blocks for small M. A debug workspace-range query is also added.

```diff
diff --git a/include/plbert.h b/include/plbert.h
--- a/include/plbert.h
+++ b/include/plbert.h
@@ -156,6 +156,7 @@
 void plb_set_gemm_nt_tile(int tile);
 void plb_set_gemm_nt_prefetch(int on);
 void plb_set_attn_bwd_fused(int on);
+int plb_debug_ws_range(const PlbEngine* e, int32_t which, int64_t* offset, int64_t* bytes);
 void plb_set_prune_last(int on);
 
 #ifdef __cplusplus
diff --git a/plbert_amd/_lib.py b/plbert_amd/_lib.py
--- a/plbert_amd/_lib.py
+++ b/plbert_amd/_lib.py
@@ -49,7 +49,7 @@
     "plb_packing_plan", "plb_forward_packed", "plb_loss_fwd_bwd_packed", "plb_loss_fwd_packed", "plb_encode", "plb_encode_bwd", "plb_status", "plb_status_ex", "plb_poll_status", "plb_status_export", "plb_status_import", "plb_broadcast_params", "plb_set_grad_overlap", "plb_allreduce_grads", "plb_apply_mask",
     "plb_mask_batch", "plb_profile_enable", "plb_profile_num_classes", "plb_profile_class_name", "plb_profile_read",
     "plb_debug_skip_piece", "plb_debug_ln_fault", "plb_debug_hb_audit", "plb_debug_hb_report", "plb_comm_trace", "plb_comm_trace_read",
-    "plb_set_gemm_nt_tile", "plb_set_gemm_nt_prefetch", "plb_set_attn_bwd_fused", "plb_set_prune_last",
+    "plb_set_gemm_nt_tile", "plb_set_gemm_nt_prefetch", "plb_set_attn_bwd_fused", "plb_set_prune_last", "plb_debug_ws_range",
 ]
 
 
@@ -234,6 +234,9 @@
     L.plb_comm_trace_read.argtypes = [vp, i32, C.POINTER(i32), i64p, i64p, C.POINTER(f32), C.POINTER(f32), C.POINTER(f32)]
     L.plb_debug_ln_fault.restype = None
     L.plb_debug_ln_fault.argtypes = [C.c_int, C.c_int]
+    if hasattr(L, "plb_debug_ws_range"):
+        L.plb_debug_ws_range.restype = C.c_int
+        L.plb_debug_ws_range.argtypes = [vp, i32, i64p, i64p]
     L.plb_debug_skip_piece.restype = None
     L.plb_debug_skip_piece.argtypes = [C.c_int]
     L.plb_comm_pieces.restype = C.c_int
diff --git a/plbert_amd/csrc/attn_bwd_fused.hip b/plbert_amd/csrc/attn_bwd_fused.hip
--- a/plbert_amd/csrc/attn_bwd_fused.hip
+++ b/plbert_amd/csrc/attn_bwd_fused.hip
@@ -414,11 +414,11 @@
   if (p->row_start && !p->lengths) return 1;
   if (p->ldqkv % 8 || p->ldctx % 8 || p->lddctx % 8 || p->lddqkv % 8) return 1;
   if ((!p->dqkv && !p->dqkv8) || (p->dqkv8 && (!p->dqkv_scale || p->lddqkv8 % 8))) return 1;
+  if (p->dqkv && p->dqkv8) return 1;
   dim3 grid(p->NH * p->B), block(256);
   const double unit = (double)p->B * p->NH * (double)p->S * p->S * 64.0;
   const double io = 2.0 * p->B * p->S * (double)p->H;
   const int tok = plb_prof_begin(PLB_K_ATTN_BWD, stream, 8.0 * unit, 6.0 * io);
-  if (p->dqkv && p->dqkv8) return 1;
   if (!p->dqkv8) hipLaunchKernelGGL(attn_bwd_fused_kernel<0>, grid, block, 0, stream, *p);
   else hipLaunchKernelGGL(attn_bwd_fused_kernel<1>, grid, block, 0, stream, *p);
   plb_prof_end(tok, stream);
diff --git a/plbert_amd/csrc/engine.cpp b/plbert_amd/csrc/engine.cpp
--- a/plbert_amd/csrc/engine.cpp
+++ b/plbert_amd/csrc/engine.cpp
@@ -129,6 +129,7 @@
   e->o_rows = cv.take(NM * 4); e->o_tgt = cv.take(NM * 4); e->o_w = cv.take(NM * 4); e->o_lrows = cv.take(NM * 4);
   if (tr) {
     e->o_dhm = cv.take(NM * H * 2);
+    e->o_inv = cv.take(Tp * 4);
     int64_t slab = 0;
     {
       const int64_t Mtot = L * Tp;
@@ -223,6 +224,12 @@
 }
 
 extern "C" int64_t plb_workspace_bytes(const PlbEngine* e) { return e ? e->ws_bytes : -1; }
+extern "C" int plb_debug_ws_range(const PlbEngine* e, int32_t which, int64_t* offset, int64_t* bytes) {
+  if (!e || e->infer || !offset || !bytes || which < 0 || which > 1) return 1;
+  *offset = which == 0 ? e->o_dctx : e->o_da;
+  *bytes = e->Tcap * e->H * 2;
+  return 0;
+}
 
 extern "C" int plb_bind(PlbEngine* e, float* params, float* grads, float* exp_avg, float* exp_avg_sq, void* workspace,
                         int64_t workspace_bytes) {
diff --git a/plbert_amd/csrc/engine_calls.cpp b/plbert_amd/csrc/engine_calls.cpp
--- a/plbert_amd/csrc/engine_calls.cpp
+++ b/plbert_amd/csrc/engine_calls.cpp
@@ -331,7 +331,7 @@
   if (n_masked == 0 && !token_targets) return zero_loss_call(e, backward, loss, s);
 
   const int NM = (int)rup(n_masked, 128);
-  Prune pr = {e->at<int32_t>(e->o_rows), n_masked, NM};
+  Prune pr = {e->at<int32_t>(e->o_rows), n_masked, NM, nullptr};
   const bool prune = prune_enabled() && n_masked > 0 && !token_targets && e->L >= 2 && 2 * (int64_t)NM <= Tp;
   if (n_masked > 0) {
     if (rw.row_start)
@@ -340,6 +340,10 @@
     else
       TRY(plb_launch_ce_prepare(idx_offsets, idx_flat, labels, B, S, e->at<int32_t>(e->o_rows), e->at<int32_t>(e->o_tgt),
                                 e->at<float>(e->o_w), s));
+  }
+  if (prune && backward) {
+    pr.inv = e->at<int32_t>(e->o_inv);
+    TRY(plb_launch_inverse_rows(pr.rows, n_masked, (int)Tp, e->at<int32_t>(e->o_inv), s));
   }
   if (backward) e->pruned_rows = prune ? NM : 0;
   e->last_app_rows[0] = prune ? NM : Tp; e->last_app_rows[1] = Tp;
diff --git a/plbert_amd/csrc/engine_internal.h b/plbert_amd/csrc/engine_internal.h
--- a/plbert_amd/csrc/engine_internal.h
+++ b/plbert_amd/csrc/engine_internal.h
@@ -80,7 +80,7 @@
   int64_t o_lse, o_delta, o_mean1, o_rstd1, o_mean2, o_rstd2;
   int64_t o_dqkv, o_dpre1, o_du, o_dpre2;
   int64_t o_dy0, o_dy1, o_da, o_dctx, o_de;
-  int64_t o_hm, o_logm, o_dlog, o_dhm, o_rows, o_tgt, o_w, o_lrows;
+  int64_t o_hm, o_logm, o_dlog, o_dhm, o_rows, o_tgt, o_w, o_lrows, o_inv = 0;
   int64_t o_slab, o_part1, o_part2, o_parte, o_scratch, o_dxe, o_ducol, o_slab2, o_scratch2, o_qkvcol = 0;
   int64_t o_lnx = 0, o_lnerr = 0;
   int64_t o_bt = 0, o_wtT = 0, o_tdl = 0, o_tlrows = 0, o_tscr = 0, o_tgrad = 0, o_tloss = 0;
@@ -174,7 +174,7 @@
 
 struct LnSlot { const float* gamma; const float* beta; const bf16_t* pre; float* mean; float* rstd; float* partials; };
 
-struct Prune { const int32_t* rows; int n; int Mc; };
+struct Prune { const int32_t* rows; int n; int Mc; const int32_t* inv; };
 
 struct Bwd {
   const int32_t* lengths;
diff --git a/plbert_amd/csrc/engine_layers.cpp b/plbert_amd/csrc/engine_layers.cpp
--- a/plbert_amd/csrc/engine_layers.cpp
+++ b/plbert_amd/csrc/engine_layers.cpp
@@ -164,8 +164,7 @@
   bf16_t* xc = stash ? e->at<bf16_t>(e->o_da) : sl.a;
   bf16_t* pre1c = stash ? sl.pre1 : sl.ctx;
   bf16_t* ac = stash ? sl.a : sl.pre1;
-  TRY(plb_launch_gather_rows(ctx_att, H, pr->rows, n, Mc, H, ctxc, H, s));
-  TRY(plb_launch_gather_rows(sl.x, H, pr->rows, n, Mc, H, xc, H, s));
+  TRY(plb_launch_gather_rows2(ctx_att, sl.x, H, pr->rows, n, Mc, H, ctxc, xc, H, s));
   PlbGemmNT g = nt_desc(ctxc, e->wbf(PLB_DENSE_W), Mc, H, H);
   g.bias = e->par(PLB_DENSE_B); g.res = xc; g.ldr = H; g.C = pre1c; g.ldc = H;
   const LnSlot ln1 = {e->par(PLB_LN1_W), e->par(PLB_LN1_B), pre1c, sl.mean1, sl.rstd1, nullptr};
@@ -378,10 +377,8 @@
   g = nt_desc(sl.dpre1, e->at<bf16_t>(e->o_wdT), Mc, H, H);
   g.C = dctxc; g.ldc = H;
   TRY(plb_launch_gemm_nt(&g, 0, 0, s));
-  HIPTRY(hipMemsetAsync(dctx, 0, (size_t)c.Tp * H * 2, s));
-  TRY(plb_launch_scatter_rows(dctxc, H, pr->rows, n, H, dctx, H, s));
-  HIPTRY(hipMemsetAsync(dac, 0, (size_t)c.Tp * H * 2, s));
-  TRY(plb_launch_scatter_rows(sl.dpre1, H, pr->rows, n, H, dac, H, s));
+  if (!pr->inv) return fail("last_application_bwd_pruned: no inverse row map");
+  TRY(plb_launch_scatter_fill_rows(dctxc, sl.dpre1, H, pr->inv, n, (int)c.Tp, H, dctx, dac, H, s));
   return 0;
 }
 
diff --git a/plbert_amd/csrc/gemm.hip b/plbert_amd/csrc/gemm.hip
--- a/plbert_amd/csrc/gemm.hip
+++ b/plbert_amd/csrc/gemm.hip
@@ -8,9 +8,10 @@
 
 DEVI int nt_lds_off(int row, int chunk) { return row * BK + ((chunk ^ ((row >> 1) & 7)) << 3); }
 
-template <int ACT, bool OUTF32>
+template <int ACT, bool OUTF32, int TBM>
 __global__ __launch_bounds__(256) void gemm_nt_kernel(PlbGemmNT p) {
-  __shared__ __attribute__((aligned(16))) bf16_t smem[2][2][BM * BK];
+  constexpr int MI = TBM / 32;
+  __shared__ __attribute__((aligned(16))) bf16_t smem[2][(TBM + BN) * BK];
   const int tid = threadIdx.x, lane = tid & 63, wave = tid >> 6;
   const int wr = wave >> 1, wc = wave & 1;
   const int nbn = (p.N + BN - 1) / BN;
@@ -20,7 +21,7 @@
 
   const int uw = __builtin_amdgcn_readfirstlane(wave);
   const int drow = lane >> 3, dch = lane & 7;
-  const bf16_t* gA = p.A + (size_t)(bm * BM + uw * 32 + drow) * p.lda;
+  const bf16_t* gA = p.A + (size_t)(bm * TBM + uw * (8 * MI) + drow) * p.lda;
   const bf16_t* gB = p.B + (size_t)(bn * BN + uw * 32 + drow) * p.ldb;
   const size_t sa = (size_t)8 * p.lda, sb = (size_t)8 * p.ldb;
   int sch[4];
@@ -31,35 +32,35 @@
 #define NT_STAGE(st, kt)                                                                              \
   do {                                                                                                \
     _Pragma("unroll") for (int i = 0; i < 4; ++i) {                                                   \
-      __builtin_amdgcn_global_load_lds((gptr_t)(gA + i * sa + (size_t)(kt) * BK + sch[i]),            \
-                                       (lptr_t)&smem[st][0][(uw * 32 + i * 8) * BK], 16, 0, 0);       \
+      if (i < MI)                                                                                     \
+        __builtin_amdgcn_global_load_lds((gptr_t)(gA + i * sa + (size_t)(kt) * BK + sch[i]),          \
+                                         (lptr_t)&smem[st][(uw * (8 * MI) + i * 8) * BK], 16, 0, 0);  \
       __builtin_amdgcn_global_load_lds((gptr_t)(gB + i * sb + (size_t)(kt) * BK + sch[i]),            \
-                                       (lptr_t)&smem[st][1][(uw * 32 + i * 8) * BK], 16, 0, 0);       \
+                                       (lptr_t)&smem[st][(TBM + uw * 32 + i * 8) * BK], 16, 0, 0);    \
     }                                                                                                 \
   } while (0)
 #define NT_LANDED() asm volatile("s_waitcnt vmcnt(0)" ::: "memory")
 
-  f32x4 acc[4][4];
-#pragma unroll
-  for (int i = 0; i < 4; ++i)
+  f32x4 acc[MI][4];
+#pragma unroll
+  for (int i = 0; i < MI; ++i)
 #pragma unroll
     for (int j = 0; j < 4; ++j) acc[i][j] = f32x4{0.f, 0.f, 0.f, 0.f};
 
   const int frow = lane & 15, fq = lane >> 4;
   const int fsw = (frow >> 1) & 7;
-  const int offA = (wr * 64 + frow) * BK, offB = (wc * 64 + frow) * BK;
+  const int offA = (wr * (16 * MI) + frow) * BK, offB = (TBM + wc * 64 + frow) * BK;
 #define NT_COMPUTE(st)                                                                                   \
   do {                                                                                                   \
-    const bf16_t* sA = smem[st][0];                                                                      \
-    const bf16_t* sB = smem[st][1];                                                                      \
+    const bf16_t* sT = smem[st];                                                                         \
     _Pragma("unroll") for (int kk = 0; kk < 2; ++kk) {                                                   \
       const int ch = ((kk * 4 + fq) ^ fsw) << 3;                                                         \
-      bf16x8 af[4], bfr[4];                                                                              \
+      bf16x8 af[MI], bfr[4];                                                                             \
       _Pragma("unroll") for (int i = 0; i < 4; ++i) {                                                    \
-        af[i] = *(const bf16x8*)&sA[offA + i * 16 * BK + ch];                                            \
-        bfr[i] = *(const bf16x8*)&sB[offB + i * 16 * BK + ch];                                           \
+        if (i < MI) af[i] = *(const bf16x8*)&sT[offA + i * 16 * BK + ch];                                \
+        bfr[i] = *(const bf16x8*)&sT[offB + i * 16 * BK + ch];                                           \
       }                                                                                                  \
-      _Pragma("unroll") for (int mi = 0; mi < 4; ++mi)                                                   \
+      _Pragma("unroll") for (int mi = 0; mi < MI; ++mi)                                                  \
         _Pragma("unroll") for (int ni = 0; ni < 4; ++ni)                                                 \
           acc[mi][ni] = __builtin_amdgcn_mfma_f32_16x16x32_bf16(bfr[ni], af[mi], acc[mi][ni], 0, 0, 0);  \
     }                                                                                                    \
@@ -81,8 +82,8 @@
 #undef NT_COMPUTE
 
 #pragma unroll
-  for (int mi = 0; mi < 4; ++mi) {
-    const int m = bm * BM + wr * 64 + mi * 16 + frow;
+  for (int mi = 0; mi < MI; ++mi) {
+    const int m = bm * TBM + wr * (16 * MI) + mi * 16 + frow;
 #pragma unroll
     for (int ni = 0; ni < 4; ++ni)
       nt_epilogue<ACT, OUTF32>(p, acc[mi][ni], m, bn * BN + wc * 64 + ni * 16 + fq * 4);
@@ -192,7 +193,7 @@
 static int pick_tile(const PlbGemmNT* p) {
   const bool ok256 = p->M % 256 == 0 && p->N % 256 == 0, ok384 = p->M % 128 == 0 && p->N % 384 == 0;
   const bool ok1256 = p->M % 128 == 0 && p->N % 256 == 0;
-  if (g_nt_tile == 128) return 128;
+  if (g_nt_tile == 128 || g_nt_tile == 64) return 128;
   if (g_nt_tile == 256) return ok256 ? 256 : 128;
   if (g_nt_tile == 384) return ok384 ? 384 : (ok256 ? 256 : 128);
   if (g_nt_tile == 1256) return ok1256 ? 1256 : 128;
@@ -213,13 +214,38 @@
   return tile == 256 ? 2 * (M / 256) : (tile == 384 || tile == 1256) ? 2 * (M / 128) : 0;
 }
 
+static int small_rows(const PlbGemmNT* p) {
+  if (g_nt_tile == 64) return p->M % 64 == 0 ? 64 : 128;
+  return p->M % BM ? 64 : 128;
+}
+
+template <int TBM>
+static int launch_small(const PlbGemmNT* p, int act, int out_f32, dim3 grid, hipStream_t stream) {
+  const dim3 block(256);
+  if (out_f32) {
+    if (act != 0) return 1;
+    hipLaunchKernelGGL((gemm_nt_kernel<0, true, TBM>), grid, block, 0, stream, *p);
+  } else if (act == 0) {
+    hipLaunchKernelGGL((gemm_nt_kernel<0, false, TBM>), grid, block, 0, stream, *p);
+  } else if (act == 1) {
+    hipLaunchKernelGGL((gemm_nt_kernel<1, false, TBM>), grid, block, 0, stream, *p);
+  } else if (act == 2) {
+    hipLaunchKernelGGL((gemm_nt_kernel<2, false, TBM>), grid, block, 0, stream, *p);
+  } else {
+    return 1;
+  }
+  return 0;
+}
+
 extern "C" int plb_launch_gemm_nt(const PlbGemmNT* p, int act, int out_f32, hipStream_t stream) {
-  if (p->M % BM || p->K % BK || p->N % 4 || p->M <= 0 || p->N <= 0 || p->K <= 0) return 1;
+  if (p->M % 64 || p->K % BK || p->N % 4 || p->M <= 0 || p->N <= 0 || p->K <= 0) return 1;
   const int nbn = (p->N + BN - 1) / BN;
-  dim3 grid((p->M / BM) * nbn), block(256);
   const int cls = out_f32 ? PLB_K_GEMM_NT_F32 : act == 1 ? PLB_K_GEMM_NT_GELU : act == 2 ? PLB_K_GEMM_NT_GELUBWD : PLB_K_GEMM_NT;
-  const int tile = pick_tile(p);
+  const int tile = p->M % BM ? 128 : pick_tile(p);
+  const int rows = tile == 128 ? small_rows(p) : 0;
+  if (tile == 128 && p->M % rows) return 1;
   if (p->colpart && tile == 128) return 1;
+  if (tile == 128 && (out_f32 ? act != 0 : (act < 0 || act > 2))) return 1;
   const double mnk = (double)p->M * p->N * p->K;
   const double algo_bytes = 2.0 * ((double)p->M * p->K + (double)p->N * p->K) +
                             (double)p->M * p->N * (out_f32 ? 4 : act == 1 ? 4 : 2) +
@@ -231,18 +257,9 @@
     return rc;
   }
   const int tok = plb_prof_begin(out_f32 ? PLB_K_GEMM_NT_F32 : PLB_K_GEMM_NT_SMALL, stream, 2.0 * mnk, algo_bytes);
-  if (out_f32) {
-    if (act != 0) return 1;
-    hipLaunchKernelGGL((gemm_nt_kernel<0, true>), grid, block, 0, stream, *p);
-  } else if (act == 0) {
-    hipLaunchKernelGGL((gemm_nt_kernel<0, false>), grid, block, 0, stream, *p);
-  } else if (act == 1) {
-    hipLaunchKernelGGL((gemm_nt_kernel<1, false>), grid, block, 0, stream, *p);
-  } else if (act == 2) {
-    hipLaunchKernelGGL((gemm_nt_kernel<2, false>), grid, block, 0, stream, *p);
-  } else {
-    return 1;
-  }
+  const dim3 grid((p->M / rows) * nbn);
+  if (rows == 64) launch_small<64>(p, act, out_f32, grid, stream);
+  else launch_small<128>(p, act, out_f32, grid, stream);
   plb_prof_end(tok, stream);
   return hipGetLastError() == hipSuccess ? 0 : 2;
 }
diff --git a/plbert_amd/csrc/plbert_kernels.h b/plbert_amd/csrc/plbert_kernels.h
--- a/plbert_amd/csrc/plbert_kernels.h
+++ b/plbert_amd/csrc/plbert_kernels.h
@@ -151,6 +151,11 @@
                            int ldd, hipStream_t stream);
 int plb_launch_scatter_rows(const bf16_t* src, int lds_, const int32_t* rows, int n, int H, bf16_t* dst, int ldd,
                             hipStream_t stream);
+int plb_launch_gather_rows2(const bf16_t* src0, const bf16_t* src1, int lds_, const int32_t* rows, int n, int npad, int H,
+                            bf16_t* dst0, bf16_t* dst1, int ldd, hipStream_t stream);
+int plb_launch_inverse_rows(const int32_t* rows, int n, int Tp, int32_t* inv, hipStream_t stream);
+int plb_launch_scatter_fill_rows(const bf16_t* src0, const bf16_t* src1, int lds_, const int32_t* inv, int n, int Tp, int H,
+                                 bf16_t* dst0, bf16_t* dst1, int ldd, hipStream_t stream);
 int plb_launch_ce_prepare(const int32_t* offsets, const int32_t* flat, const int64_t* labels, int B, int S,
                           int32_t* rows, int32_t* tgt, float* w, hipStream_t stream);
 int plb_launch_ce_prepare_packed(const int32_t* offsets, const int32_t* flat, const int64_t* labels, int B, int S,
diff --git a/plbert_amd/csrc/rowops.hip b/plbert_amd/csrc/rowops.hip
--- a/plbert_amd/csrc/rowops.hip
+++ b/plbert_amd/csrc/rowops.hip
@@ -721,6 +721,46 @@
   for (int c = threadIdx.x; c < H / 8; c += blockDim.x)
     *(uint4*)(dst + drow * ldd + c * 8) = *(const uint4*)(src + (size_t)r * lds_ + c * 8);
 }
+__global__ void gather_rows2_kernel(const bf16_t* src0, const bf16_t* src1, int lds_, const int32_t* rows, int n, int H,
+                                    bf16_t* dst0, bf16_t* dst1, int ldd) {
+  const bf16_t* src = blockIdx.y ? src1 : src0;
+  bf16_t* dst = blockIdx.y ? dst1 : dst0;
+  const int r = blockIdx.x;
+  const int chunks = H / 8;
+  const bool live = r < n;
+  const size_t srow = live ? (size_t)rows[r] : 0;
+  for (int c = threadIdx.x; c < chunks; c += blockDim.x) {
+    uint4 v = live ? *(const uint4*)(src + srow * lds_ + c * 8) : make_uint4(0, 0, 0, 0);
+    *(uint4*)(dst + (size_t)r * ldd + c * 8) = v;
+  }
+}
+__global__ __launch_bounds__(256) void inverse_rows_kernel(const int32_t* rows, int n, int Tp, int32_t* inv) {
+  __shared__ int own[256];
+  const int base = blockIdx.x * 256;
+  own[threadIdx.x] = -1;
+  __syncthreads();
+  for (int j = threadIdx.x; j < n; j += 256) {
+    const unsigned d = (unsigned)(rows[j] - base);
+    if (d < 256u) atomicMax(&own[d], j);
+  }
+  __syncthreads();
+  if (base + (int)threadIdx.x < Tp) inv[base + threadIdx.x] = own[threadIdx.x];
+}
+__global__ __launch_bounds__(256) void scatter_fill_rows_kernel(const bf16_t* src0, const bf16_t* src1, int lds_,
+                                                                const int32_t* inv, int n, int Tp, int H, bf16_t* dst0,
+                                                                bf16_t* dst1, int ldd) {
+  const int lane = threadIdx.x & 63, wave = threadIdx.x >> 6;
+  const int t = blockIdx.x * 4 + wave;
+  if (t >= Tp) return;
+  const bf16_t* src = blockIdx.y ? src1 : src0;
+  bf16_t* dst = blockIdx.y ? dst1 : dst0;
+  const int j = inv[t];
+  const bool live = j >= 0 && j < n;
+  for (int c = lane; c < H / 8; c += 64) {
+    uint4 v = live ? *(const uint4*)(src + (size_t)j * lds_ + c * 8) : make_uint4(0, 0, 0, 0);
+    *(uint4*)(dst + (size_t)t * ldd + c * 8) = v;
+  }
+}
 __global__ void ce_prepare_kernel(const int32_t* offsets, const int32_t* flat, const int64_t* labels, int B, int S,
                                   const int32_t* row_start, int32_t* rows, int32_t* tgt, float* w) {
   __shared__ int cnt[4];
@@ -1178,6 +1218,28 @@
 , dim3(n), dim3(128), 0, stream, src, lds_, rows, n, H, dst, ldd);
   return LAUNCH_OK();
 }
+extern "C" int plb_launch_gather_rows2(const bf16_t* src0, const bf16_t* src1, int lds_, const int32_t* rows, int n,
+                                       int npad, int H, bf16_t* dst0, bf16_t* dst1, int ldd, hipStream_t stream) {
+  if (H % 8 || npad <= 0 || n > npad || !src0 || !dst0 || !src1 != !dst1) return 1;
+  const int pairs = src1 ? 2 : 1;
+  ProfScope ps(PLB_K_ROWS, stream, 0, 4.0 * (double)pairs * npad * H);
+  hipLaunchKernelGGL(gather_rows2_kernel, dim3(npad, pairs), dim3(128), 0, stream, src0, src1, lds_, rows, n, H, dst0, dst1, ldd);
+  return LAUNCH_OK();
+}
+extern "C" int plb_launch_inverse_rows(const int32_t* rows, int n, int Tp, int32_t* inv, hipStream_t stream) {
+  if (n < 0 || Tp <= 0) return 1;
+  hipLaunchKernelGGL(inverse_rows_kernel, dim3((Tp + 255) / 256), dim3(256), 0, stream, rows, n, Tp, inv);
+  return LAUNCH_OK();
+}
+extern "C" int plb_launch_scatter_fill_rows(const bf16_t* src0, const bf16_t* src1, int lds_, const int32_t* inv, int n,
+                                            int Tp, int H, bf16_t* dst0, bf16_t* dst1, int ldd, hipStream_t stream) {
+  if (H % 8 || Tp <= 0 || n < 0 || !src0 || !dst0 || !src1 != !dst1) return 1;
+  const int pairs = src1 ? 2 : 1;
+  ProfScope ps(PLB_K_ROWS, stream, 0, 2.0 * (double)pairs * ((double)Tp + n) * H);
+  hipLaunchKernelGGL(scatter_fill_rows_kernel, dim3((Tp + 3) / 4, pairs), dim3(256), 0, stream, src0, src1, lds_, inv, n, Tp,
+                     H, dst0, dst1, ldd);
+  return LAUNCH_OK();
+}
 extern "C" int plb_launch_ce_prepare(const int32_t* offsets, const int32_t* flat, const int64_t* labels, int B, int S,
                                      int32_t* rows, int32_t* tgt, float* w, hipStream_t stream) {
   hipLaunchKernelGGL(ce_prepare_kernel, dim3(B), dim3(256), 0, stream, offsets, flat, labels, B, S, nullptr, rows, tgt, w);
```

Result: no change. 1.717 million tokens/s, median of 6 (+0.2%).
